# posgraph/coupe.optical_flow_based_deep_video_stabilization

Hardware: AMD Instinct MI355X
Metric: stabilised frame-pairs/sec @512x512 (higher is better)
Workload: dtype f32; 1 GPU; batch=8 512x512x27 frame stacks per GPU: FlowNetS-pyramid forward (5 flows) + flow resize/scale + tf_warp at 512x512; batch_per_gpu=8, height=512, width=512, cin=27, all_gather=False, vgg16_trunk=False, st_warp=none, plan_flags=0, plan_batch=0, full=False

## Files before the change

### coupe/optical_flow_based_deep_video_stabilization_amd/csrc/conv1_bf16x3.hip

```cpp
#include "rowwin_tile.h"

namespace vstab {

typedef unsigned u32x2 __attribute__((ext_vector_type(2)));
typedef unsigned u32x4 __attribute__((ext_vector_type(4)));
typedef __bf16 bf16x4 __attribute__((ext_vector_type(4)));
typedef __bf16 bf16x8 __attribute__((ext_vector_type(8)));

template <int NWIN4, int MB>
__global__ __launch_bounds__(256) void conv1_bf16x3_kernel(const RowWinParams p)
{
    extern __shared__ __attribute__((aligned(16))) char smem[];
    unsigned *planes = reinterpret_cast<unsigned *>(smem);

    const RowWinTile<MB> t = rowwin_tile<MB>(p);
    const int tid = t.tid, wm = t.wm, wn = t.wn, li = t.li, lh = t.lh;
    const int oy = t.row, pix_step = t.pix_step;

    f32x4 wv[NWIN4];
    auto load_window = [&](int ky) { rowwin_load_window(t, p, oy, ky, wv); };
    const int plane_w = p.WLEN >> 1;
    auto split_store = [&]() {
#pragma unroll
        for (int j = 0; j < NWIN4; ++j) {
            const int c4 = tid + 256 * j;
            if (4 * c4 < p.WLEN) {
                bf16x4 h, m, l;
#pragma unroll
                for (int e = 0; e < 4; ++e) {
                    const float x = wv[j][e];
                    h[e] = (__bf16)x;
                    const float r1 = x - (float)h[e];
                    m[e] = (__bf16)r1;
                    const float r2 = r1 - (float)m[e];
                    l[e] = (__bf16)r2;
                }
                *reinterpret_cast<u32x2 *>(planes + 2 * c4) = __builtin_bit_cast(u32x2, h);
                *reinterpret_cast<u32x2 *>(planes + plane_w + 2 * c4) = __builtin_bit_cast(u32x2, m);
                *reinterpret_cast<u32x2 *>(planes + 2 * plane_w + 2 * c4) = __builtin_bit_cast(u32x2, l);
            }
        }
    };

    const int KG = p.SEGP >> 4;
    const int NG = p.KH * KG;
    const unsigned *bbase = reinterpret_cast<const unsigned *>(p.wpk) + (wn * 32 + li) * 8 + lh * 4;
    auto load_b = [&](u32x4 (&b)[3], int G) {
        const unsigned *s = bbase + (long long)(G < NG ? G : NG - 1) * (3 * 512);
#pragma unroll
        for (int q = 0; q < 3; ++q) b[q] = *reinterpret_cast<const u32x4 *>(s + q * 512);
    };
    const int a_w0 = (pix_step * (wm * 32 * MB + li) + p.w_a + 8 * lh) >> 1;
    const int a_w1 = a_w0 + ((pix_step * 32) >> 1);
    auto load_a = [&](u32x4 (&a)[3 * MB], int g) {
#pragma unroll
        for (int mb = 0; mb < MB; ++mb)
#pragma unroll
            for (int q = 0; q < 3; ++q) {
                const unsigned *s = planes + q * plane_w + (mb ? a_w1 : a_w0) + 8 * g;
                u32x4 v;
                v.x = s[0]; v.y = s[1]; v.z = s[2]; v.w = s[3];
                a[mb * 3 + q] = v;
            }
    };

    f32x16 acc[MB];
#pragma unroll
    for (int a = 0; a < MB; ++a)
#pragma unroll
        for (int r = 0; r < 16; ++r) acc[a][r] = 0.f;

    auto mma = [&](const u32x4 (&a)[3 * MB], const u32x4 (&b)[3]) {
        constexpr int PA[6] = {2, 1, 0, 1, 0, 0}, PB[6] = {0, 1, 2, 0, 1, 0};
#pragma unroll
        for (int t = 0; t < 6; ++t)
#pragma unroll
            for (int mb = 0; mb < MB; ++mb)
                acc[mb] = __builtin_amdgcn_mfma_f32_32x32x16_bf16(__builtin_bit_cast(bf16x8, a[mb * 3 + PA[t]]),
                                                                  __builtin_bit_cast(bf16x8, b[PB[t]]), acc[mb], 0, 0, 0);
    };

    u32x4 a0[3 * MB], a1[3 * MB], b0[3], b1[3];
    load_window(0);
    load_b(b0, 0);
    split_store();
    __syncthreads();
    int G = 0;
    for (int ky = 0; ky < p.KH; ++ky) {
        const bool more = ky + 1 < p.KH;
        if (more) load_window(ky + 1);
        load_a(a0, 0);
        __builtin_amdgcn_sched_barrier(0);
        for (int g = 0; g < KG; g += 2, G += 2) {
            load_a(a1, g + 1);
            load_b(b1, G + 1);
            __builtin_amdgcn_sched_barrier(0);
            mma(a0, b0);
            __builtin_amdgcn_sched_barrier(0);
            if (g + 2 < KG) load_a(a0, g + 2);
            load_b(b0, G + 2);
            __builtin_amdgcn_sched_barrier(0);
            mma(a1, b1);
            __builtin_amdgcn_sched_barrier(0);
        }
        if (more) {
            __syncthreads();
            split_store();
            __syncthreads();
        }
    }

    rowwin_epilogue(t, p, acc, oy, reinterpret_cast<float *>(smem));
}

hipError_t conv1_bf16x3_set_attributes()
{
    return rowwin_set_lds_limits(conv1_bf16x3_kernel<7, 2>, 3 * 7 * 1024 * 2, conv1_bf16x3_kernel<4, 1>, 3 * 4 * 1024 * 2);
}

hipError_t launch_conv1_bf16x3(const RowWinParams &p, hipStream_t stream, hipEvent_t ev_start, hipEvent_t ev_stop)
{
    if (!conv1_bf16x3_geometry_ok(p)) return hipErrorInvalidValue;
    RowWinParams q = p;
    q.asm_loop = 0;
    q.stream_rows = 0;
    return rowwin_launch(q, conv1_bf16x3_kernel<7, 2>, conv1_bf16x3_kernel<4, 1>, (size_t)3 * p.WLEN * 2, stream, ev_start, ev_stop);
}

}
```

### coupe/optical_flow_based_deep_video_stabilization_amd/csrc/conv_desc.cpp

```cpp
#include <algorithm>
#include <cstring>

#include "conv_desc.h"

using namespace vstab;

namespace {
ConvParams desc_base(int B, int Hi, int Wi, int cs_in, const KLayout &L, int s_in, int s_out, int Ho, int Wo, int cout, int npad, int cs_out,
                     int c_off, int act, int nphase)
{
    ConvParams p;
    std::memset(&p, 0, sizeof p);
    p.B = B; p.Hi = Hi; p.Wi = Wi; p.Cs_in = cs_in;
    p.KH = L.KH; p.NSEG = L.NSEG; p.SEG = L.SEG; p.SEGP = L.SEGP; p.SEG_STRIDE = L.SEG_STRIDE;
    p.s_in = s_in; p.s_out = s_out; p.Ho = Ho; p.Wo = Wo; p.Cs_out = cs_out; p.c_off = c_off;
    p.N = cout; p.Npad = npad; p.act = act; p.nphase = nphase; p.ksplit = 1;
    p.in_bytes = (unsigned)std::min<long long>((long long)B * Hi * Wi * cs_in * 4, 0xFFFFFFFFLL);
    p.w_bytes = (unsigned)std::min<long long>((long long)L.ktiles() * npad * 128, 0xFFFFFFFFLL);
    return p;
}

void set_phase(ConvParams &p, int k, int Hg, int Wg, int off_y, int off_x, int o_y, int o_x)
{
    ConvPhase &ph = p.ph[k];
    ph.Hg = Hg; ph.Wg = Wg; ph.M = p.B * Hg * Wg;
    ph.off_y = off_y; ph.off_x = off_x; ph.o_y = o_y; ph.o_x = o_x;
    ph.w_off = (long long)k * ((long long)p.KH * p.NSEG * (p.SEGP / 32) * p.Npad * 32);
    p.Mmax = std::max(p.Mmax, ph.M);
}
}

ConvParams conv_desc_phase(int B, int Hi, int Wi, int cin, int cs_in, int kh, int kw, int s_in, const ConvGrid &g, int Ho, int Wo, int cout,
                           int npad, int cs_out, int c_off, int act)
{
    ConvParams p = desc_base(B, Hi, Wi, cs_in, conv_layout(kh, kw, cin, cs_in), s_in, g.s_out, Ho, Wo, cout, npad, cs_out, c_off, act, 1);
    set_phase(p, 0, g.Hg, g.Wg, g.off_y, g.off_x, g.o_y, g.o_x);
    return p;
}

ConvParams conv_desc_parity4(int B, int Hi, int Wi, int cin, int cs_in, int taps, const int off[2], int Ho, int Wo, int cout, int npad,
                             int cs_out, int c_off, int act)
{
    ConvParams p = desc_base(B, Hi, Wi, cs_in, conv_layout(taps, taps, cin, cs_in), 1, 2, Ho, Wo, cout, npad, cs_out, c_off, act, 4);
    for (int py = 0; py < 2; ++py)
        for (int px = 0; px < 2; ++px) set_phase(p, py * 2 + px, (Ho - py + 1) / 2, (Wo - px + 1) / 2, off[py], off[px], py, px);
    return p;
}

ConvParams conv_desc_planes(int B, int P, int pitch, int Wi, const int *Hg, const int *Wg, int cs_in, int cout)
{
    ConvParams p = desc_base(B, P * pitch, Wi, cs_in, klayout_run(1, 1, cs_in), 1, 1, P * pitch, Wi, cout, cout, cout, 0, 0, P);
    for (int q = 0; q < P; ++q) set_phase(p, q, Hg[q], Wg[q], q * pitch, 0, q * pitch, 0);
    return p;
}

ConvParams conv_desc_wino_gemm(int B, int H, int W, int cin, int cout)
{
    int Hg[16], Wg[16];
    for (int q = 0; q < 16; ++q) { Hg[q] = (H + 1) / 2; Wg[q] = (W + 1) / 2; }
    return conv_desc_planes(B, 16, Hg[0], Wg[0], Hg, Wg, cin, cout);
}

ConvParams conv_desc_wdec_gemm(int B, const WdecGeom &g, int cs_in, int cout)
{
    int Hg[9], Wg[9];
    for (int q = 0; q < 9; ++q) { Hg[q] = g.nty[q / 3]; Wg[q] = g.ntx[q % 3]; }
    return conv_desc_planes(B, 9, g.NTy, g.NTx, Hg, Wg, cs_in, 4 * cout);
}

RowWinDesc rowwin_desc(int B, int H, int W, int cin, int k, int stride, int pad, int Ho, int Wo, int cout, int npad, int cs_out, int c_off,
                       int act)
{
    RowWinDesc d;
    std::memset(&d, 0, sizeof d);
    RowWinParams &r = d.main;
    r.in_bytes = (unsigned)std::min<long long>((long long)B * H * W * cin * 4, 0xFFFFFFFFLL);
    r.B = B; r.Hi = H; r.Wi = W; r.Cs_in = cin; r.KH = k;
    r.SEGP = rowwin_segp(-pad, k, cin);
    r.s_in = stride; r.off_y = -pad;
    r.e_off = -pad * cin - rowwin_lead(-pad, cin);
    r.w_a = ((r.e_off % 4) + 4) % 4;
    r.Ho = Ho; r.Wo = Wo; r.Cs_out = cs_out; r.c_off = c_off; r.N = cout; r.Npad = npad; r.act = act;
    auto tile = [](RowWinParams &q, int MB) { q.MB = MB; q.WLEN = round_up(q.s_in * q.Cs_in * (64 * MB - 1) + q.w_a + q.SEGP, 4); };
    tile(r, rowwin_mb(B, Ho, Wo));
    d.ok = rowwin_geometry_ok(r);
    const int rem = Wo % 128;
    if (d.ok && r.MB == 2 && Wo > 128 && rem >= 1 && rem <= 64) {
        RowWinParams &t = d.tail;
        t = r;
        tile(t, 1);
        t.ox_base = (Wo / 128) * 128; t.ntile_x = 1;
        d.two = rowwin_geometry_ok(t);
        if (d.two) r.ntile_x = Wo / 128;
    }
    return d;
}
```

### coupe/optical_flow_based_deep_video_stabilization_amd/csrc/conv_desc.h

```cpp
#pragma once
#include "vstab_internal.h"

inline vstab::ConvTile default_tile(int cout)
{
    return cout >= 128 ? vstab::TILE_128x128 : (cout > 32 ? vstab::TILE_128x64 : vstab::TILE_128x32);
}
inline int tile_cols(vstab::ConvTile t)
{
    return (t == vstab::TILE_128x128 || t == vstab::TILE_64x128) ? 128 : ((t == vstab::TILE_128x64 || t == vstab::TILE_64x64) ? 64 : 32);
}
inline int padded_cols(int cout, vstab::ConvTile t) { return vstab::round_up(cout, tile_cols(t)); }
inline int padded_cols(int cout) { return padded_cols(cout, default_tile(cout)); }

inline vstab::KLayout conv_layout(int kh, int kw, int cin, int cs_in)
{
    return cs_in == cin ? vstab::klayout_run(kh, kw, cs_in) : vstab::klayout_tap(kh, kw, cin, cs_in);
}

struct ConvGrid { int Hg, Wg, off_y, off_x, s_out, o_y, o_x; };
vstab::ConvParams conv_desc_phase(int B, int Hi, int Wi, int cin, int cs_in, int kh, int kw, int s_in, const ConvGrid &g, int Ho, int Wo,
                                  int cout, int npad, int cs_out, int c_off, int act);
inline vstab::ConvParams conv_desc_plain(int B, int Hi, int Wi, int cin, int cs_in, int k, int stride, int pad, int Ho, int Wo, int cout,
                                         int npad, int cs_out, int c_off, int act)
{
    return conv_desc_phase(B, Hi, Wi, cin, cs_in, k, k, stride, ConvGrid{Ho, Wo, -pad, -pad, 1, 0, 0}, Ho, Wo, cout, npad, cs_out, c_off, act);
}

vstab::ConvParams conv_desc_parity4(int B, int Hi, int Wi, int cin, int cs_in, int taps, const int off[2], int Ho, int Wo, int cout, int npad,
                                    int cs_out, int c_off, int act);

vstab::ConvParams conv_desc_planes(int B, int P, int pitch, int Wi, const int *Hg, const int *Wg, int cs_in, int cout);
vstab::ConvParams conv_desc_wino_gemm(int B, int H, int W, int cin, int cout);
vstab::ConvParams conv_desc_wdec_gemm(int B, const vstab::WdecGeom &g, int cs_in, int cout);

struct RowWinDesc { vstab::RowWinParams main, tail; bool ok, two; };
RowWinDesc rowwin_desc(int B, int H, int W, int cin, int k, int stride, int pad, int Ho, int Wo, int cout, int npad, int cs_out, int c_off,
                       int act);
```

### coupe/optical_flow_based_deep_video_stabilization_amd/csrc/conv_rowwin.hip

```cpp
#include "rowwin_tile.h"

namespace vstab {

typedef float f32x2 __attribute__((ext_vector_type(2)));
typedef int i32x4 __attribute__((ext_vector_type(4)));
#include "conv_kloop_gfx950.inc"

template <int NWIN4, int MB>
__global__ __launch_bounds__(256) void conv_rowwin_kernel(const RowWinParams p)
{
    extern __shared__ __attribute__((aligned(16))) char smem[];
    float *win = reinterpret_cast<float *>(smem);

    const RowWinTile<MB> t = rowwin_tile<MB>(p);
    const int tid = t.tid, wm = t.wm, wn = t.wn, li = t.li, lh = t.lh;
    const int stream_r = (MB == 2 && p.asm_loop) ? p.stream_rows : 0;
    const int stream_s = 1;
    int oy = stream_r > 0 ? t.row * stream_r : t.row;
    const int ox0 = t.ox0, n = t.n, pix_step = t.pix_step, row_floats = t.row_floats;

    f32x4 wv[NWIN4];
    auto load_window = [&](int ky) { rowwin_load_window(t, p, oy, ky, wv); };
    constexpr int ASM_BUF = MB == 2 ? VSTAB_ROWWIN_BUF_BYTES : VSTAB_ROWWIN1_BUF_BYTES;
    const int wstride = p.asm_loop ? ASM_BUF / 4 : p.WLEN;
    auto store_window = [&](int buf) {
        float *d = win + buf * wstride;
#pragma unroll
        for (int j = 0; j < NWIN4; ++j) {
            const int c4 = tid + 256 * j;
            if (4 * c4 < p.WLEN) *reinterpret_cast<f32x4 *>(d + 4 * c4) = wv[j];
        }
    };

    const float *bbase = p.wpk + (long long)(wn * 32 + li) * 32 + lh * 4;
    const int ktile_stride = p.Npad * 32;
    f32x4 b0[4], b1[4];
    const int KT = p.KH * (p.SEGP >> 5);
    auto load_b = [&](f32x4 (&dst)[4], int kt) {
        const float *s = bbase + (long long)(kt < KT ? kt : KT - 1) * ktile_stride;
#pragma unroll
        for (int q = 0; q < 4; ++q) dst[q] = *reinterpret_cast<const f32x4 *>(s + q * 8);
    };

    f32x16 acc[MB];
#pragma unroll
    for (int a = 0; a < MB; ++a)
#pragma unroll
        for (int r = 0; r < 16; ++r) acc[a][r] = 0.f;

    const int kpr = p.SEGP >> 5;
    const int a_off0 = pix_step * (wm * 32 * MB + li) + p.w_a + 2 * lh;
    const int a_off1 = a_off0 + pix_step * 32;

    auto compute = [&](const float *w, int kc, const f32x4 (&b)[4]) {
        const float *wa0 = w + a_off0 + 32 * kc, *wa1 = w + a_off1 + 32 * kc;
#pragma unroll
        for (int r = 0; r < 8; ++r) {
            const f32x2 a0 = *reinterpret_cast<const f32x2 *>(wa0 + 4 * r);
            f32x2 a1 = a0;
            if (MB == 2) a1 = *reinterpret_cast<const f32x2 *>(wa1 + 4 * r);
#pragma unroll
            for (int j = 0; j < 2; ++j) {
                const int s = 2 * r + j;
                const float bv = b[s >> 2][s & 3];
                acc[0] = __builtin_amdgcn_mfma_f32_32x32x2f32(a0[j], bv, acc[0], 0, 0, 0);
                if (MB == 2) acc[MB - 1] = __builtin_amdgcn_mfma_f32_32x32x2f32(a1[j], bv, acc[MB - 1], 0, 0, 0);
            }
        }
    };

    load_window(0);
    store_window(0);
    if (p.asm_loop) {
        {
            __syncthreads();
            const unsigned lds0 = (unsigned)(size_t)(__attribute__((address_space(3))) void *)win;
            unsigned a0c = lds0 + (unsigned)a_off0 * 4u, a1c = lds0 + (unsigned)a_off1 * 4u;
            unsigned a0n = a0c + ASM_BUF, a1n = a1c + ASM_BUF;
            const unsigned vb = (unsigned)((wn * 32 + li) * 32 + lh * 4) * 4u;
            unsigned w[7];
#pragma unroll
            for (int j = 0; j < 7; ++j) w[j] = ROWWIN_OOB;
#pragma unroll
            for (int j = 0; j < NWIN4; ++j) {
                int g;
                if (rowwin_chunk(t, p, j, g)) w[j] = (unsigned)g * 4u;
            }
            const unsigned long long ain = (unsigned long long)(size_t)p.in, awt = (unsigned long long)(size_t)p.wpk;
            i32x4 din, dwt;
            din.x = __builtin_amdgcn_readfirstlane((int)(unsigned)ain);
            din.y = __builtin_amdgcn_readfirstlane((int)((unsigned)(ain >> 32) & 0xffffu));
            din.z = __builtin_amdgcn_readfirstlane((int)p.in_bytes);
            din.w = 0x00020000;
            dwt.x = __builtin_amdgcn_readfirstlane((int)(unsigned)awt);
            dwt.y = __builtin_amdgcn_readfirstlane((int)((unsigned)(awt >> 32) & 0xffffu));
            dwt.z = __builtin_amdgcn_readfirstlane(KT * ktile_stride * 4);
            dwt.w = 0x00020000;
            const int wave_u = __builtin_amdgcn_readfirstlane(tid) >> 6;
            const int m_cur = __builtin_amdgcn_readfirstlane((int)lds0 + wave_u * 1024);
            int m_n = m_cur + ASM_BUF;
            const int m_x = m_cur ^ m_n;
            int s_iy = oy * p.s_in + p.off_y + 1;
            int s_soff = ((n * p.Hi + s_iy) * p.Wi) * p.Cs_in * 4;
            int s_koff = 0, s_nrows = p.KH - 1;
            unsigned v_t0, v_t1;
            long long s_mask;
            if (MB == 2 && stream_r > 0) {
                const unsigned long long aout = (unsigned long long)(size_t)p.out;
                i32x4 dout;
                dout.x = __builtin_amdgcn_readfirstlane((int)(unsigned)aout);
                dout.y = __builtin_amdgcn_readfirstlane((int)((unsigned)(aout >> 32) & 0xffffu));
                dout.z = __builtin_amdgcn_readfirstlane((int)((unsigned)p.B * (unsigned)p.Ho * (unsigned)p.Wo * (unsigned)p.Cs_out * 4u));
                dout.w = 0x00020000;
                const unsigned vout = (unsigned)((wm * 64 + 4 * lh) * p.Cs_out + p.c_off + wn * 32 + li) * 4u;
                const float bias_l = p.bias[wn * 32 + li];
                const float slope = p.act == 1 ? 0.1f : (p.act == 0 ? 1.0f : 0.0f);
                int s_ntiles = stream_r, s_obase = (((n * p.Ho + oy) * p.Wo + ox0) * p.Cs_out) * 4, s_st;
                float o[32];
                asm volatile(VSTAB_ROWWIN_STREAM_ASM_KPR6
                             : [a0c] "+v"(a0c), [a1c] "+v"(a1c), [a0n] "+v"(a0n), [a1n] "+v"(a1n),
                               [mn] "+s"(m_n), [iy] "+s"(s_iy), [soff] "+s"(s_soff), [koff] "+s"(s_koff), [nrows] "+s"(s_nrows), [ntiles] "+s"(s_ntiles),
                               [obase] "+s"(s_obase), [st] "=&s"(s_st), [vt0] "=&v"(v_t0), [vt1] "=&v"(v_t1), [mask] "=&s"(s_mask),
                               [o0] "=&v"(o[0]), [o1] "=&v"(o[1]), [o2] "=&v"(o[2]), [o3] "=&v"(o[3]), [o4] "=&v"(o[4]), [o5] "=&v"(o[5]), [o6] "=&v"(o[6]),
                               [o7] "=&v"(o[7]), [o8] "=&v"(o[8]), [o9] "=&v"(o[9]), [o10] "=&v"(o[10]), [o11] "=&v"(o[11]), [o12] "=&v"(o[12]),
                               [o13] "=&v"(o[13]), [o14] "=&v"(o[14]), [o15] "=&v"(o[15]), [o16] "=&v"(o[16]), [o17] "=&v"(o[17]), [o18] "=&v"(o[18]),
                               [o19] "=&v"(o[19]), [o20] "=&v"(o[20]), [o21] "=&v"(o[21]), [o22] "=&v"(o[22]), [o23] "=&v"(o[23]), [o24] "=&v"(o[24]),
                               [o25] "=&v"(o[25]), [o26] "=&v"(o[26]), [o27] "=&v"(o[27]), [o28] "=&v"(o[28]), [o29] "=&v"(o[29]), [o30] "=&v"(o[30]),
                               [o31] "=&v"(o[31])
                             : [vb] "v"(vb), [w0] "v"(w[0]), [w1] "v"(w[1]), [w2] "v"(w[2]), [w3] "v"(w[3]), [w4] "v"(w[4]), [w5] "v"(w[5]), [w6] "v"(w[6]),
                               [din] "s"(din), [dwt] "s"(dwt), [mx] "s"(m_x), [hi] "s"(p.Hi), [rowbytes] "s"(row_floats * 4), [kstride] "s"(ktile_stride * 4),
                               [bias] "v"(bias_l), [slope] "s"(slope), [cs4] "s"(p.Cs_out * 4), [ostep] "s"(stream_s * p.Wo * p.Cs_out * 4), [vout] "v"(vout),
                               [dout] "s"(dout), [fwd] "s"(stream_s * p.s_in - p.KH)
                             : "memory", "scc", VSTAB_ROWWIN_STREAM_CLOBBERS);
#pragma unroll
                for (int r = 0; r < 16; ++r) { acc[0][r] = o[r]; acc[MB - 1][r] = o[16 + r]; }
                oy += (stream_r - 1) * stream_s;
            } else if constexpr (MB == 1) {
                asm volatile(VSTAB_ROWWIN1_ASM_KPR6
                             : [c0] "+a"(acc[0]), [a0c] "+v"(a0c), [a0n] "+v"(a0n),
                               [mn] "+s"(m_n), [iy] "+s"(s_iy), [soff] "+s"(s_soff), [koff] "+s"(s_koff), [nrows] "+s"(s_nrows),
                               [vt0] "=&v"(v_t0), [vt1] "=&v"(v_t1), [mask] "=&s"(s_mask)
                             : [vb] "v"(vb), [w0] "v"(w[0]), [w1] "v"(w[1]), [w2] "v"(w[2]), [w3] "v"(w[3]),
                               [din] "s"(din), [dwt] "s"(dwt), [mx] "s"(m_x), [hi] "s"(p.Hi), [rowbytes] "s"(row_floats * 4), [kstride] "s"(ktile_stride * 4)
                             : "memory", "scc", VSTAB_ROWWIN1_CLOBBERS);
                (void)a1c; (void)a1n;
            } else
            asm volatile(VSTAB_ROWWIN_ASM_KPR6
                         : [c0] "+a"(acc[0]), [c1] "+a"(acc[MB - 1]), [a0c] "+v"(a0c), [a1c] "+v"(a1c), [a0n] "+v"(a0n), [a1n] "+v"(a1n),
                           [mn] "+s"(m_n), [iy] "+s"(s_iy), [soff] "+s"(s_soff), [koff] "+s"(s_koff), [nrows] "+s"(s_nrows),
                           [vt0] "=&v"(v_t0), [vt1] "=&v"(v_t1), [mask] "=&s"(s_mask)
                         : [vb] "v"(vb), [w0] "v"(w[0]), [w1] "v"(w[1]), [w2] "v"(w[2]), [w3] "v"(w[3]), [w4] "v"(w[4]), [w5] "v"(w[5]), [w6] "v"(w[6]),
                           [din] "s"(din), [dwt] "s"(dwt), [mx] "s"(m_x), [hi] "s"(p.Hi), [rowbytes] "s"(row_floats * 4), [kstride] "s"(ktile_stride * 4)
                         : "memory", "scc", VSTAB_ROWWIN_CLOBBERS);
        }
    } else {
    load_b(b0, 0);
    __syncthreads();
    int buf = 0, kt = 0;
    for (int ky = 0; ky < p.KH; ++ky) {
        const bool more = ky + 1 < p.KH;
        if (more) load_window(ky + 1);
        __builtin_amdgcn_sched_barrier(0);
        const float *w = win + buf * p.WLEN;
        int kc = 0;
        for (; kc + 1 < kpr; kc += 2, kt += 2) {
            load_b(b1, kt + 1);
            __builtin_amdgcn_sched_barrier(0);
            compute(w, kc, b0);
            load_b(b0, kt + 2);
            __builtin_amdgcn_sched_barrier(0);
            compute(w, kc + 1, b1);
        }
        if (kc < kpr) {
            load_b(b1, kt + 1);
            __builtin_amdgcn_sched_barrier(0);
            compute(w, kc, b0);
#pragma unroll
            for (int q = 0; q < 4; ++q) b0[q] = b1[q];
            ++kt;
        }
        if (more) {
            store_window(buf ^ 1);
            __syncthreads();
            buf ^= 1;
        }
    }
    }

    rowwin_epilogue(t, p, acc, oy, win);
}

hipError_t rowwin_set_attributes()
{
    return rowwin_set_lds_limits(conv_rowwin_kernel<7, 2>, 2 * 7 * 1024 * 4, conv_rowwin_kernel<4, 1>, 2 * 4 * 1024 * 4);
}

hipError_t launch_conv_rowwin(const RowWinParams &p, hipStream_t stream, hipEvent_t ev_start, hipEvent_t ev_stop)
{
    const int ntx = rowwin_xtiles(p);
    if (!rowwin_geometry_ok(p) || ntx < 0) return hipErrorInvalidValue;
    RowWinParams q = p;
    q.asm_loop = ((p.SEGP >> 5) == 6 && p.KH >= 1 && 4 * p.WLEN <= (p.MB == 2 ? VSTAB_ROWWIN_BUF_BYTES : VSTAB_ROWWIN1_BUF_BYTES)) ? 1 : 0;
#ifdef VSTAB_NO_ASM_KLOOP
    q.asm_loop = 0;
#endif
    q.stream_rows = 0;
    if (q.asm_loop && p.MB == 2 && p.KH == 7 && p.N == 64 && p.act >= 0 && p.act <= 2 && p.ox_base + ntx * 128 <= p.Wo &&
        (unsigned long long)p.B * p.Ho * p.Wo * p.Cs_out * 4ull < 0x80000000ull) {
        const double F = 0.08;
        const long long cols = (long long)ntx * p.B;
        double best = (double)((cols * p.Ho + 511) / 512) * (1.0 + F);
        for (int R = 2; R <= 32 && R <= p.Ho; ++R) {
            if (p.Ho % R) continue;
            const long long wgs = cols * (p.Ho / R);
            const double c = wgs <= 256 ? 0.53 * R + F : (double)((wgs + 511) / 512) * (R + F);
            if (c < best * 0.995) { best = c; q.stream_rows = R; }
        }
    }
#ifdef VSTAB_NO_ROWWIN_STREAM
    q.stream_rows = 0;
#endif
    const size_t lds2 = q.asm_loop ? (size_t)2 * (p.MB == 2 ? VSTAB_ROWWIN_BUF_BYTES : VSTAB_ROWWIN1_BUF_BYTES) : (size_t)2 * p.WLEN * 4;
    return rowwin_launch(q, conv_rowwin_kernel<7, 2>, conv_rowwin_kernel<4, 1>, lds2, stream, ev_start, ev_stop);
}

}
```

### coupe/optical_flow_based_deep_video_stabilization_amd/csrc/flownet_forward.cpp

```cpp
#include <cmath>
#include <cstdlib>
#include <memory>

#include "flownet_plan.h"

using namespace vstab;

static const char *UP_NAME[4] = {"upsample6_5", "upsample5_4", "upsample4_3", "upsample3_2"};

extern "C" int vstab_load_weights(vstab_ctx *ctx, const vstab_tensor *t, int count)
{
    if (!ctx) return fail(nullptr, VSTAB_E_STATE, "vstab_load_weights: ctx is NULL");
    if (!t || count <= 0) return fail(ctx, VSTAB_E_WEIGHTS, "vstab_load_weights: no tensors");
    const vstab_tensor *w1 = find(t, count, "1/W_conv2d");
    if (!w1 || w1->ndim != 4) return fail(ctx, VSTAB_E_WEIGHTS, "missing variable 1/W_conv2d");
    const int cin = w1->shape[2];
    if (cin < 1 || cin > 4096) return fail(ctx, VSTAB_E_WEIGHTS, "1/W_conv2d: bad Cin %d", cin);

    std::vector<float> host;
    auto reserve = [&](size_t n) { size_t o = (host.size() + 63) / 64 * 64; host.resize(o + n, 0.f); return o; };
    std::vector<double> scale;
    auto need = [&](const std::string &name, std::initializer_list<int> s) -> const vstab_tensor * {
        const vstab_tensor *x = find(t, count, name);
        return shape_is(x, s) ? x : nullptr;
    };
#define NEED(var, name, ...)                                                                   \
    const vstab_tensor *var = need(name, {__VA_ARGS__});                                        \
    if (!var) return fail(ctx, VSTAB_E_WEIGHTS, "missing or mis-shaped variable %s", std::string(name).c_str());

    for (int i = 0; i < 10; ++i) {
        const Layer &e = NET[i];
        const int ci = i == 0 ? cin : e.cin;
        const int cs_in = i == 0 ? cin : in_buf(e).cs;
        const std::string n = e.name + 4;
        NEED(W, n + "/W_conv2d", e.k, e.k, ci, e.cout)
        NEED(b, n + "/b_conv2d", e.cout)
        NEED(beta, n + "/beta", e.cout)
        NEED(mean, n + "/moving_mean", e.cout)
        NEED(var, n + "/moving_variance", e.cout)
        const int npad = padded_cols(e.cout);
        const KLayout L = conv_layout(e.k, e.k, ci, cs_in);
        scale.assign(npad, 1.0);
        ctx->enc_b[i] = reserve(npad);
        fold_bn(b->data, beta->data, mean->data, var->data, e.cout, npad, scale.data(), host.data() + ctx->enc_b[i]);
        ctx->enc_w[i] = reserve((size_t)L.ktiles() * npad * 32);
        pack_conv(W->data, scale.data(), e.k, e.k, ci, cs_in, e.cout, npad, L, host.data() + ctx->enc_w[i]);
        if (e.k == 3 && e.s == 1 && (ci & 31) == 0 && (e.cout & 127) == 0) {
            ctx->wino_w[i] = reserve((size_t)16 * (ci / 32) * e.cout * 32);
            pack_winograd(W->data, scale.data(), ci, e.cout, e.cout, host.data() + ctx->wino_w[i]);
        }
        if (i == 0) {
            const int lead = rowwin_lead(-e.p, cin), segp = rowwin_segp(-e.p, e.k, cin);
            ctx->enc0_rw = reserve((size_t)e.k * (segp / 32) * npad * 32);
            pack_conv_rowwin(W->data, scale.data(), e.k, e.k, cin, e.cout, npad, lead, segp, host.data() + ctx->enc0_rw);
            ctx->enc0_b3 = 0;
            if (npad == 64) {
                ctx->enc0_b3 = reserve((size_t)e.k * (segp / 16) * 3 * 64 * 16 / 2);
                pack_conv1_bf16x3(W->data, scale.data(), e.k, e.k, cin, e.cout, lead, segp, reinterpret_cast<uint16_t *>(host.data() + ctx->enc0_b3));
            }
        }
    }
    for (int l = 0; l < 4; ++l) {
        const Layer &d = dec_layer(l);
        const std::string n = d.name;
        const int co = d.cout, ci = d.cin, cs = in_buf(d).cs;
        NEED(W, n + "/W_deconv2d", 4, 4, co, ci)
        NEED(b, n + "/b_deconv2d", co)
        NEED(beta, n + "_bn/beta", co)
        NEED(mean, n + "_bn/moving_mean", co)
        NEED(var, n + "_bn/moving_variance", co)
        const int npad = padded_cols(co);
        scale.assign(npad, 1.0);
        ctx->dec_b[l] = reserve(npad);
        fold_bn(b->data, beta->data, mean->data, var->data, co, npad, scale.data(), host.data() + ctx->dec_b[l]);
        ctx->dec_w[l] = reserve(4 * (size_t)klayout_deconv(cs).ktiles() * npad * 32);
        pack_deconv(W->data, scale.data(), ci, cs, co, npad, host.data() + ctx->dec_w[l]);
        ctx->wdec_w[l] = 0;
        if (l <= 2) {
            ctx->wdec_w[l] = reserve(9 * (size_t)klayout_run(1, 1, cs).ktiles() * 4 * co * 32);
            pack_wdec(W->data, scale.data(), ci, cs, co, host.data() + ctx->wdec_w[l]);
        }

        const std::string u = UP_NAME[l];
        NEED(uw, u + "/W_deconv2d", 4, 4, 2, 2)
        NEED(ub, u + "/b_deconv2d", 2)
        std::memcpy(ctx->up[l].w, uw->data, sizeof(float) * 64);
        ctx->up[l].b[0] = ub->data[0]; ctx->up[l].b[1] = ub->data[1];
    }
    for (int l = 0; l < 4; ++l) {
        const Layer &h = head_layer(l);
        const std::string n = h.name;
        NEED(W, n + "/W_conv2d", 3, 3, h.cin, 2)
        NEED(b, n + "/b_conv2d", 2)
        ctx->pred_w[l] = reserve((size_t)klayout_run(1, 1, in_buf(h).cs).ktiles() * 32 * 32);
        pack_predict2_table(W->data, h.cin, in_buf(h).cs, 32, host.data() + ctx->pred_w[l]);
        ctx->pred_b[l] = reserve(4);
        host[ctx->pred_b[l]] = b->data[0]; host[ctx->pred_b[l] + 1] = b->data[1];
    }
    {
        NEED(W, "predict2/W_conv2d", 3, 3, NET[14].cin, 2)
        NEED(b, "predict2/b_conv2d", 2)
        ctx->tab_b = reserve(32);
        ctx->tab_wp = reserve((size_t)200 * 32);
        pack_predict2_panel(W->data, NET[14].cin, 200, host.data() + ctx->tab_wp);
        ctx->zero_b = reserve(2048);
        ctx->pred2_b = reserve(4);
        host[ctx->pred2_b] = b->data[0]; host[ctx->pred2_b + 1] = b->data[1];
    }
#undef NEED

    HIP_TRY(ctx, hipSetDevice(ctx->device));
    if (ctx->dev_weights) { (void)hipFree(ctx->dev_weights); ctx->dev_weights = nullptr; }
    ctx->loaded = false;
    hipError_t e = hipMalloc(reinterpret_cast<void **>(&ctx->dev_weights), host.size() * sizeof(float));
    if (e != hipSuccess) return fail(ctx, VSTAB_E_NOMEM, "hipMalloc(%zu bytes of packed weights): %s", host.size() * 4, hipGetErrorString(e));
    HIP_TRY(ctx, hipMemcpy(ctx->dev_weights, host.data(), host.size() * sizeof(float), hipMemcpyHostToDevice));
    ctx->dev_weight_floats = host.size();
    ctx->cin = cin;
    ctx->loaded = true;
    return VSTAB_OK;
}

struct FusedTail { const float *frame; float *outflow; float *warped; int oh, ow; bool fused; const uint8_t *frame8; uint8_t *out8; };
static int forward_chunk(vstab_ctx *ctx, const float *feats, int B, int H, int W, int Cin, float *pf6, float *pf5,
                         float *pf4, float *pf3, float *pf2, void *workspace, size_t workspace_bytes, void *stream_, FusedTail *tail);
static const char *conv_kernel_name(ConvTile t, bool vec4);
static const char *dual_kernel_name(ConvTile t);
static int forward_impl(vstab_ctx *ctx, const float *feats, int B, int H, int W, int Cin, float *pf6, float *pf5, float *pf4, float *pf3,
                        float *pf2, void *workspace, size_t workspace_bytes, void *stream_, FusedTail *tail);

extern "C" int vstab_flownets_forward(vstab_ctx *ctx, const float *feats, int B, int H, int W, int Cin, float *pf6,
                                      float *pf5, float *pf4, float *pf3, float *pf2, void *workspace,
                                      size_t workspace_bytes, void *stream_)
{
    return forward_impl(ctx, feats, B, H, W, Cin, pf6, pf5, pf4, pf3, pf2, workspace, workspace_bytes, stream_, nullptr);
}

static int forward_impl(vstab_ctx *ctx, const float *feats, int B, int H, int W, int Cin, float *pf6, float *pf5, float *pf4, float *pf3,
                        float *pf2, void *workspace, size_t workspace_bytes, void *stream_, FusedTail *tail)
{
    if (!ctx) return fail(nullptr, VSTAB_E_STATE, "forward: ctx is NULL");
    if (!ctx->loaded) return fail(ctx, VSTAB_E_STATE, "forward: vstab_load_weights has not been called");
    if (Cin != ctx->cin) return fail(ctx, VSTAB_E_SHAPE, "forward: feats has %d channels, weights expect %d", Cin, ctx->cin);
    if (!feats || !pf6 || !pf5 || !pf4 || !pf3 || !pf2 || !workspace) return fail(ctx, VSTAB_E_STATE, "forward: NULL buffer");
    int eh[10], ew[10];
    if (B < 1 || !level_sizes(H, W, eh, ew)) return fail(ctx, VSTAB_E_SHAPE, "forward: unsupported problem %dx%dx%dx%d", B, H, W, Cin);
    const PlanPin pin = pin_of(ctx);
    if (pin.batch > 0 && B > pin.batch) return fail(ctx, VSTAB_E_SHAPE, "forward: batch %d exceeds the pinned plan batch %d (vstab_set_plan_batch)", B, pin.batch);
    const int chunk = chunk_size(pin, B, H, W, Cin);
    if (chunk < 1) return fail(ctx, VSTAB_E_SHAPE, "forward: one %dx%dx%d sample exceeds the 2 GiB tensor limit", H, W, Cin);
    bool all_fused = tail != nullptr && (chunk >= B || ((size_t)tail->oh * tail->ow * 4) % 16 == 0);
    for (int b0 = 0; b0 < B; b0 += chunk) {
        const int bc = std::min(chunk, B - b0);
        FusedTail t{};
        if (tail && all_fused) {
            const size_t px = (size_t)b0 * tail->oh * tail->ow;
            t = FusedTail{tail->frame ? tail->frame + px * 3 : nullptr, tail->outflow ? tail->outflow + px * 2 : nullptr,
                          tail->warped ? tail->warped + px * 3 : nullptr, tail->oh, tail->ow, false,
                          tail->frame8 ? tail->frame8 + px * 3 : nullptr, tail->out8 ? tail->out8 + px * 3 : nullptr};
        }
        const int rc = forward_chunk(ctx, feats + (size_t)b0 * H * W * Cin, bc, H, W, Cin,
                                     pf6 + (size_t)b0 * eh[9] * ew[9] * 2, pf5 + (size_t)b0 * eh[7] * ew[7] * 2,
                                     pf4 + (size_t)b0 * eh[5] * ew[5] * 2, pf3 + (size_t)b0 * eh[3] * ew[3] * 2,
                                     pf2 + (size_t)b0 * (H - 2) * (W - 2) * 2, workspace, workspace_bytes, stream_, (tail && all_fused) ? &t : nullptr);
        if (rc != VSTAB_OK) return rc;
        if (tail && all_fused && !t.fused) {
            if (b0 != 0) return fail(ctx, VSTAB_E_ALIGN, "stabilise: chunk %d of the batch misses the fused tail's alignment", b0 / chunk);
            all_fused = false;
        }
    }
    if (tail) tail->fused = all_fused;
    return VSTAB_OK;
}

static int conv1_rowwin(vstab_ctx *ctx, bool bf16x3, const float *feats, int B, int H, int W, int Cin, int Ho, int Wo, int N, int Npad,
                        float *out, int cs_out, int c_off, unsigned *tickets, hipStream_t stream, hipEvent_t ev_a, hipEvent_t ev_b,
                        const char **kname, bool *launched)
{
    const Layer &e = NET[0];
    const float *dw = ctx->dev_weights;
    *launched = false;
    RowWinDesc d = rowwin_desc(B, H, W, Cin, e.k, e.s, e.p, Ho, Wo, N, Npad, cs_out, c_off, 1);
    if (!d.ok || ((uintptr_t)feats & 15) != 0) return VSTAB_OK;
    const bool b3 = bf16x3 && ctx->enc0_b3 != 0 && conv1_bf16x3_geometry_ok(d.main);
    RowWinParams &r = d.main, &t = d.tail;
    r.in = t.in = feats; r.out = t.out = out; r.bias = t.bias = dw + ctx->enc_b[0];
    r.wpk = t.wpk = dw + (b3 ? ctx->enc0_b3 : ctx->enc0_rw);
    auto launch1 = [&](const RowWinParams &q, hipEvent_t a, hipEvent_t b) {
        return b3 ? launch_conv1_bf16x3(q, stream, a, b) : launch_conv_rowwin(q, stream, a, b);
    };
    if (tickets) { r.clear_words = tickets; r.clear_n = SKINNY_MAX_TILES; }
    *launched = true;
    if (d.two) {
        HIP_TRY(ctx, launch1(r, ev_a, nullptr));
        HIP_TRY(ctx, launch1(t, nullptr, ev_b));
        *kname = b3 ? "conv1_bf16x3_kernel<7, 2> + <4, 1> tail" : "conv_rowwin_kernel<7, 2> + <4, 1> tail";
        return VSTAB_OK;
    }
    HIP_TRY(ctx, launch1(r, ev_a, ev_b));
    if (b3) *kname = r.MB == 2 ? "conv1_bf16x3_kernel<7, 2>" : "conv1_bf16x3_kernel<4, 1>";
    else *kname = r.MB == 2 ? "conv_rowwin_kernel<7, 2>" : "conv_rowwin_kernel<4, 1>";
    return VSTAB_OK;
}

extern "C" int vstab_conv1_forward(vstab_ctx *ctx, const float *feats, int B, int H, int W, int Cin, float *out, int cs_out, int c_off,
                                   void *stream_)
{
    if (!ctx) return fail(nullptr, VSTAB_E_STATE, "conv1_forward: ctx is NULL");
    if (!ctx->loaded) return fail(ctx, VSTAB_E_STATE, "conv1_forward: vstab_load_weights has not been called");
    if (Cin != ctx->cin) return fail(ctx, VSTAB_E_SHAPE, "conv1_forward: feats has %d channels, weights expect %d", Cin, ctx->cin);
    if (!feats || !out) return fail(ctx, VSTAB_E_STATE, "conv1_forward: NULL buffer");
    const PlanPin pin = pin_of(ctx);
    std::unique_ptr<Plan> pl(new (std::nothrow) Plan);
    if (!pl) return fail(ctx, VSTAB_E_NOMEM, "conv1_forward: out of host memory");
    if (B < 1 || !make_plan(B, H, W, Cin, *pl, &pin)) return fail(ctx, VSTAB_E_SHAPE, "conv1_forward: unsupported problem %dx%dx%dx%d", B, H, W, Cin);
    const ConvParams &p = pl->cp[0];
    if (c_off < 0 || cs_out < c_off + p.N || (long long)B * p.Ho * p.Wo * cs_out * 4 >= 0x80000000LL)
        return fail(ctx, VSTAB_E_SHAPE, "conv1_forward: output slice %d + %d of %d channels", c_off, p.N, cs_out);
    if (((uintptr_t)feats & 15) || ((uintptr_t)out & 3)) return fail(ctx, VSTAB_E_ALIGN, "conv1_forward: feats must be 16-byte aligned");
    const char *kname = nullptr;
    bool launched = false;
    const int rc = conv1_rowwin(ctx, pl->conv1_bf16x3, feats, B, H, W, Cin, p.Ho, p.Wo, p.N, p.Npad, out, cs_out, c_off, nullptr,
                                (hipStream_t)stream_, nullptr, nullptr, &kname, &launched);
    if (rc != VSTAB_OK) return rc;
    if (!launched) return fail(ctx, VSTAB_E_SHAPE, "conv1_forward: the row-window kernels do not take this geometry");
    return VSTAB_OK;
}

static int forward_chunk(vstab_ctx *ctx, const float *feats, int B, int H, int W, int Cin, float *pf6, float *pf5,
                         float *pf4, float *pf3, float *pf2, void *workspace, size_t workspace_bytes, void *stream_, FusedTail *tail)
{
    Plan pl;
    const PlanPin pin = pin_of(ctx);
    if (!make_plan(B, H, W, Cin, pl, &pin)) return fail(ctx, VSTAB_E_SHAPE, "forward: unsupported problem %dx%dx%dx%d", B, H, W, Cin);
    if (workspace_bytes < pl.total) return fail(ctx, VSTAB_E_NOMEM, "forward: workspace %zu < %zu bytes", workspace_bytes, pl.total);
    if (((uintptr_t)workspace & 255) != 0) return fail(ctx, VSTAB_E_ALIGN, "forward: workspace must be 256-byte aligned");
    if (((uintptr_t)feats & 15) || ((uintptr_t)pf6 & 7) || ((uintptr_t)pf5 & 7) || ((uintptr_t)pf4 & 7) ||
        ((uintptr_t)pf3 & 7) || ((uintptr_t)pf2 & 7))
        return fail(ctx, VSTAB_E_ALIGN, "forward: feats must be 16-byte and flows 8-byte aligned");
    hipStream_t stream = (hipStream_t)stream_;
    char *ws = (char *)workspace;
    auto buf = [&](int b) { return (float *)(ws + pl.off[b]); };
    const float *dw = ctx->dev_weights;
    unsigned *tickets = reinterpret_cast<unsigned *>(buf(B_TICKETS));
    bool any_tickets = false;
    for (int i = 0; i < 14; ++i) any_tickets = any_tickets || (pl.skinny[i] && pl.cp[i].ksplit > 1);
    bool tickets_cleared = !any_tickets;

    hipEvent_t *ev = nullptr;
    if (ctx->prof) {
        const size_t need = (size_t)(ctx->prof_forwards + 1) * 30;
        while (ctx->prof_ev.size() < need) {
            hipEvent_t e;
            HIP_TRY(ctx, hipEventCreate(&e));
            ctx->prof_ev.push_back(e);
        }
        ev = ctx->prof_ev.data() + (size_t)ctx->prof_forwards * 30;
        for (int i = 0; i < 15; ++i) {
            const ConvParams &p = pl.cp[i];
            double mac = 0;
            if (i < 10 && pl.wino[i]) mac = 16.0 * pl.wcp[i].Mmax * NET[i].cin * p.N;
            else if (i < 10) mac = (double)p.ph[0].M * NET[i].k * NET[i].k * (i == 0 ? Cin : NET[i].cin) * p.N;
            else if (i < 14 && pl.wdec[i - 10]) {
                for (int k = 0; k < 9; ++k) mac += (double)pl.wdcp[i - 10].ph[k].M * NET[i].cin * 4.0 * p.N;
            }
            else if (i < 14) mac = (double)B * p.Ho * p.Wo * 4.0 * NET[i].cin * p.N;
            else mac = (double)p.ph[0].M * 194.0 * 18.0;
            ctx->prof_flops[i] += 2.0 * mac;
            double dmac = mac;
            if (i < 10 && pl.wino[i]) dmac = (double)p.ph[0].M * 9.0 * NET[i].cin * p.N;
            if (i >= 10 && i < 14 && pl.wdec[i - 10]) dmac = (double)B * p.Ho * p.Wo * 4.0 * NET[i].cin * p.N;
            ctx->prof_flops_direct[i] += 2.0 * dmac;
        }
    }
#define PROF_NAME(slot, name) do { if (ev) ctx->prof_kernel[slot] = (name); } while (0)
#define EV_A(slot) (ev ? ev[2 * (slot)] : nullptr)
#define EV_B(slot) (ev ? ev[2 * (slot) + 1] : nullptr)

    static const char *const HEAD_RANGE[4] = {"predict_flow6+upsample6_5", "predict_flow5+upsample5_4", "predict_flow4+upsample4_3", "predict_flow3+upsample3_2"};
    TraceRange whole_range("flownetS_pyramid");
    for (int i = 0; i < 10; ++i) {
        const Layer &e = NET[i];
        TraceRange layer_range(e.name);
        ConvParams p = pl.cp[i];
        if (i == 0) {
            const char *kname = nullptr;
            bool launched = false;
            const int rc = conv1_rowwin(ctx, pl.conv1_bf16x3, feats, B, H, W, Cin, p.Ho, p.Wo, p.N, p.Npad, buf(B_CONV1), p.Cs_out, 0,
                                        tickets_cleared ? nullptr : tickets, stream, EV_A(0), EV_B(0), &kname, &launched);
            if (rc != VSTAB_OK) return rc;
            if (launched) { tickets_cleared = true; PROF_NAME(0, kname); continue; }
        }
        if (!tickets_cleared) { HIP_TRY(ctx, hipMemsetAsync(tickets, 0, pl.bytes[B_TICKETS], stream)); tickets_cleared = true; }
        if (pl.wino[i]) {
            ConvParams q = pl.wcp[i];
            const int cin_i = e.cin;
            HIP_TRY(ctx, launch_wino_input(buf(e.in), B, pl.eh[i], pl.ew[i], in_buf(e).cs, 0, cin_i, buf(B_WINO_V), stream));
            q.in = buf(B_WINO_V); q.out = buf(B_WINO_M);
            q.wpk = dw + ctx->wino_w[i]; q.bias = dw + ctx->zero_b; q.partial = buf(B_PARTIAL);
            const int T_i = ((pl.eh[i] + 1) / 2) * ((pl.ew[i] + 1) / 2);
            const int P_i = wino_gemm_stream_positions(B, T_i, cin_i, e.cout);
            if (P_i > 0) {
                HIP_TRY(ctx, launch_wino_gemm_stream(q.in, q.wpk, q.out, B, T_i, cin_i, e.cout, P_i, stream, EV_A(i), EV_B(i)));
                PROF_NAME(i, "wino_gemm_stream_kernel");
            } else {
                HIP_TRY(ctx, launch_conv(q, pl.wtile[i], true, stream, EV_A(i), EV_B(i)));
                PROF_NAME(i, conv_kernel_name(pl.wtile[i], true));
            }
            HIP_TRY(ctx, launch_wino_output(buf(B_WINO_M), B, pl.eh[i], pl.ew[i], e.cout, dw + ctx->enc_b[i], 1, buf(e.out),
                                            out_buf(e).cs, 0, stream));
            continue;
        }
        p.in = e.in < 0 ? feats : buf(e.in);
        p.out = buf(e.out);
        p.wpk = dw + ctx->enc_w[i];
        p.bias = dw + ctx->enc_b[i];
        p.partial = buf(B_PARTIAL);
        if (pl.skinny[i]) {
            HIP_TRY(ctx, launch_conv_skinny(p, tickets, stream, EV_A(i), EV_B(i)));
            PROF_NAME(i, "conv_skinny_kernel<1, 4>");
            continue;
        }
        HIP_TRY(ctx, launch_conv(p, pl.tile[i], pl.vec4[i], stream, EV_A(i), EV_B(i)));
        PROF_NAME(i, conv_kernel_name(pl.tile[i], pl.vec4[i]));
    }
    float *pfs[5] = {pf6, pf5, pf4, pf3, pf2};
    for (int l = 0; l < 4; ++l) {
        const float *prev = l == 0 ? nullptr : pfs[l - 1];
        const Layer &d = dec_layer(l);
        const int ph_ = l == 0 ? 0 : pl.eh[LVL_ENC[l - 1]], pw_ = l == 0 ? 0 : pl.ew[LVL_ENC[l - 1]];
        const int oh = pl.eh[LVL_ENC[l + 1]], ow = pl.ew[LVL_ENC[l + 1]];
        ConvParams pd = pl.cp[10 + l], pt = pl.cp[15 + l];
        pd.in = buf(d.in); pd.out = buf(d.out);
        pd.wpk = dw + ctx->dec_w[l]; pd.bias = dw + ctx->dec_b[l]; pd.partial = buf(B_PARTIAL);
        const size_t dec_slab = pd.ksplit > 1 ? (size_t)pd.nphase * pd.ksplit * pd.Mmax * pd.Npad : 0;
        pt.in = buf(head_layer(l).in); pt.out = buf(head_layer(l).out);
        pt.wpk = dw + ctx->pred_w[l]; pt.bias = dw + ctx->tab_b; pt.partial = buf(B_PARTIAL) + dec_slab;
        const float *tsrc = pt.ksplit > 1 ? pt.partial : pt.out;
        const bool fuse = !(pin.flags & VSTAB_PLAN_NO_DUAL) && !pl.skinny[10 + l];
        auto head = [&](const float *taps, const ConvParams *combine, const WdecOutArgs *wdec) {
            return launch_predict_up(taps, pt.ksplit, (long long)pt.Mmax * pt.Npad, B, pt.Hi, pt.Wi, dw + ctx->pred_b[l], prev, ph_, pw_, pfs[l],
                                     ctx->up[l], buf(d.out), oh, ow, out_buf(d).cs, out_buf(d).c - 2, stream, combine, wdec);
        };
        auto dual = [&](const ConvParams &a, ConvTile ta) -> int {
            const hipError_t e = launch_conv_dual(a, ta, pt, pl.tile[15 + l], stream, EV_A(10 + l), EV_B(10 + l));
            if (e == hipErrorNotSupported) {
                HIP_TRY(ctx, launch_conv(pt, pl.tile[15 + l], true, stream, nullptr, nullptr, false));
                HIP_TRY(ctx, launch_conv(a, ta, true, stream, EV_A(10 + l), EV_B(10 + l), false));
                PROF_NAME(10 + l, conv_kernel_name(ta, true));
            } else {
                HIP_TRY(ctx, e);
                PROF_NAME(10 + l, dual_kernel_name(ta));
            }
            return VSTAB_OK;
        };
        if (fuse && pl.wdec[l]) {
            const WdecGeom &g = pl.wdg[l];
            {
                TraceRange r2(d.name);
                HIP_TRY(ctx, launch_wdec_input(pd.in, B, pd.Hi, pd.Wi, pd.Cs_in, buf(B_WINO_V), g, stream));
                ConvParams q = pl.wdcp[l];
                q.in = buf(B_WINO_V); q.out = buf(B_WINO_M); q.wpk = dw + ctx->wdec_w[l]; q.bias = dw + ctx->zero_b; q.partial = buf(B_PARTIAL);
                pt.partial = buf(B_PARTIAL);
                if (const int rc = dual(q, pl.wdtile[l])) return rc;
            }
            TraceRange r3(HEAD_RANGE[l]);
            const WdecOutArgs wo{buf(B_WINO_M), pd.N / 4, dw + ctx->dec_b[l], 1, buf(d.out), pd.Ho, pd.Wo, pd.Cs_out, pd.c_off, g};
            HIP_TRY(ctx, head(pt.ksplit > 1 ? pt.partial : pt.out, nullptr, &wo));
            continue;
        }
        if (fuse) {
            {
                TraceRange r2(d.name);
                if (const int rc = dual(pd, pl.tile[10 + l])) return rc;
            }
            TraceRange r3(HEAD_RANGE[l]);
            HIP_TRY(ctx, head(tsrc, &pd, nullptr));
            continue;
        }
        {
            TraceRange head_range(HEAD_RANGE[l]);
            HIP_TRY(ctx, launch_conv(pt, pl.tile[15 + l], true, stream, nullptr, nullptr, false));
            HIP_TRY(ctx, head(tsrc, nullptr, nullptr));
        }
        TraceRange layer_range(d.name);
        if (pl.skinny[10 + l]) {
            HIP_TRY(ctx, launch_conv_skinny(pd, tickets, stream, EV_A(10 + l), EV_B(10 + l)));
            PROF_NAME(10 + l, "conv_skinny_kernel<1, 4>");
        } else {
            HIP_TRY(ctx, launch_conv(pd, pl.tile[10 + l], true, stream, EV_A(10 + l), EV_B(10 + l)));
            PROF_NAME(10 + l, conv_kernel_name(pl.tile[10 + l], true));
        }
    }
    {
        TraceRange layer_range("predict_flow2");
        ConvParams p = pl.cp[14];
        p.in = buf(B_CONCAT2); p.out = buf(B_T);
        const long long M2 = (long long)B * pl.eh[1] * pl.ew[1];
        if (!tap_panel_applicable(M2, p.Cs_in, p.in, p.out)) return fail(ctx, VSTAB_E_SHAPE, "predict_flow2 tap table: unsupported geometry");
        HIP_TRY(ctx, launch_tap_panel(p.in, M2, dw + ctx->tab_wp, p.out, stream, EV_A(14), EV_B(14)));
        PROF_NAME(14, "tap_panel_kernel");
        hipError_t te = hipErrorNotSupported;
        if (tail && !(pin.flags & VSTAB_PLAN_NO_TAIL)) {
            TraceRange tail_range("predict_flow2 gather+flow_glue+tf_warp");
            if (tail->frame8)
                te = launch_pf2_glue_warp_u8(buf(B_T), B, pl.eh[1], pl.ew[1], dw + ctx->pred2_b, pf3, pl.eh[3], pl.ew[3], pf2, H, W, tail->frame8,
                                             tail->outflow, tail->out8, tail->oh, tail->ow, stream);
            else
                te = launch_pf2_glue_warp(buf(B_T), B, pl.eh[1], pl.ew[1], dw + ctx->pred2_b, pf3, pl.eh[3], pl.ew[3], pf2, H, W, tail->frame,
                                          tail->outflow, tail->warped, tail->oh, tail->ow, stream);
            if (te != hipSuccess && te != hipErrorNotSupported) HIP_TRY(ctx, te);
            tail->fused = te == hipSuccess;
        }
        if (te != hipSuccess) HIP_TRY(ctx, launch_pf2(buf(B_T), B, pl.eh[1], pl.ew[1], dw + ctx->pred2_b, pf3, pl.eh[3], pl.ew[3], pf2, H, W, stream));
    }
#undef EV_A
#undef EV_B
#undef PROF_NAME
    if (ev) ctx->prof_forwards++;
    return VSTAB_OK;
}

static const char *conv_kernel_name(ConvTile t, bool vec4)
{
    const bool dma = conv_uses_lds_dma(t, vec4);
#define VSTAB_KN(shape) (vec4 ? (dma ? "conv_mfma_kernel<" shape ", true, true>" : "conv_mfma_kernel<" shape ", true, false>") \
                              : (dma ? "conv_mfma_kernel<" shape ", false, true>" : "conv_mfma_kernel<" shape ", false, false>"))
    switch (t) {
    case TILE_128x128: return VSTAB_KN("128, 128, 2, 2");
    case TILE_128x64: return VSTAB_KN("128, 64, 2, 2");
    case TILE_64x128: return VSTAB_KN("64, 128, 1, 4");
    case TILE_64x64: return VSTAB_KN("64, 64, 2, 2");
    case TILE_256x32: return VSTAB_KN("256, 32, 4, 1");
    default: return VSTAB_KN("128, 32, 4, 1");
    }
#undef VSTAB_KN
}

static const char *dual_kernel_name(ConvTile t)
{
    const bool dma = conv_uses_lds_dma(t, true);
#define VSTAB_DN(shape) (dma ? "conv_dual_kernel: conv_mfma_kernel<" shape ", true, true> + <128, 32> tap table" \
                             : "conv_dual_kernel: conv_mfma_kernel<" shape ", true, false> + <128, 32> tap table")
    switch (t) {
    case TILE_128x128: return VSTAB_DN("128, 128, 2, 2");
    case TILE_128x64: return VSTAB_DN("128, 64, 2, 2");
    case TILE_64x128: return VSTAB_DN("64, 128, 1, 4");
    case TILE_64x64: return VSTAB_DN("64, 64, 2, 2");
    case TILE_256x32: return VSTAB_DN("256, 32, 4, 1");
    default: return VSTAB_DN("128, 32, 4, 1");
    }
#undef VSTAB_DN
}

extern "C" int vstab_profile_kernel_name(vstab_ctx *ctx, int slot, char *buf, int cap)
{
    if (!ctx || !buf || cap < 1 || slot < 0 || slot > 14) return fail(ctx, VSTAB_E_STATE, "profile_kernel_name: bad argument");
    std::snprintf(buf, (size_t)cap, "%s", ctx->prof_kernel[slot] ? ctx->prof_kernel[slot] : "");
    return VSTAB_OK;
}

extern "C" int vstab_profile_enable(vstab_ctx *ctx, int enable)
{
    if (!ctx) return fail(nullptr, VSTAB_E_STATE, "profile_enable: ctx is NULL");
    ctx->prof = enable != 0;
    return VSTAB_OK;
}

extern "C" int vstab_profile_reset(vstab_ctx *ctx)
{
    if (!ctx) return fail(nullptr, VSTAB_E_STATE, "profile_reset: ctx is NULL");
    ctx->prof_forwards = 0;
    for (double &f : ctx->prof_flops) f = 0;
    for (double &f : ctx->prof_flops_direct) f = 0;
    return VSTAB_OK;
}

extern "C" int vstab_profile_read(vstab_ctx *ctx, double *ms_sum15, double *flops15, int *n_forwards)
{
    if (!ctx || !ms_sum15 || !flops15 || !n_forwards) return fail(ctx, VSTAB_E_STATE, "profile_read: NULL argument");
    for (int i = 0; i < 15; ++i) { ms_sum15[i] = 0; flops15[i] = ctx->prof_flops[i]; }
    for (int f = 0; f < ctx->prof_forwards; ++f)
        for (int i = 0; i < 15; ++i) {
            float ms = 0.f;
            HIP_TRY(ctx, hipEventElapsedTime(&ms, ctx->prof_ev[(size_t)f * 30 + 2 * i], ctx->prof_ev[(size_t)f * 30 + 2 * i + 1]));
            ms_sum15[i] += ms;
        }
    *n_forwards = ctx->prof_forwards;
    return VSTAB_OK;
}

extern "C" int vstab_profile_read_direct(vstab_ctx *ctx, double *flops15)
{
    if (!ctx || !flops15) return fail(ctx, VSTAB_E_STATE, "profile_read_direct: NULL argument");
    for (int i = 0; i < 15; ++i) flops15[i] = ctx->prof_flops_direct[i];
    return VSTAB_OK;
}

extern "C" int vstab_stabilise_originalsize(vstab_ctx *ctx, const float *feats, int B, int H, int W, int Cin, const float *frame, int oh,
                                            int ow, float *pf6, float *pf5, float *pf4, float *pf3, float *pf2, float *outflow,
                                            float *warped, void *workspace, size_t workspace_bytes, void *stream)
{
    if (!frame || !warped) return fail(ctx, VSTAB_E_STATE, "stabilise_originalsize: NULL buffer");
    if (oh < 1 || ow < 1) return fail(ctx, VSTAB_E_SHAPE, "stabilise_originalsize: bad output size");
    FusedTail tail{frame, outflow, warped, oh, ow, false, nullptr, nullptr};
    const bool try_fused = (((uintptr_t)frame | (uintptr_t)warped | (uintptr_t)outflow) & 15) == 0;
    const int rc = forward_impl(ctx, feats, B, H, W, Cin, pf6, pf5, pf4, pf3, pf2, workspace, workspace_bytes, stream, try_fused ? &tail : nullptr);
    if (rc != VSTAB_OK) return rc;
    if (tail.fused) return VSTAB_OK;
    const int rc2 = vstab_flow_glue_warp(pf2, B, H - 2, W - 2, frame, outflow, warped, oh, ow, 3, H, W, stream);
    if (rc2 != VSTAB_OK) adopt_last_error(ctx);
    return rc2;
}

extern "C" int vstab_clip_step(vstab_ctx *ctx, const uint8_t *const *slots8, const uint8_t *frame, int n, int net_h, int net_w, int oh, int ow,
                               float *feats, float *pf6, float *pf5, float *pf4, float *pf3, float *pf2, float *outflow, uint8_t *out,
                               uint8_t *ring_slot, void *workspace, size_t workspace_bytes, void *stream)
{
    if (!ctx) return fail(nullptr, VSTAB_E_STATE, "clip_step: ctx is NULL");
    if (!slots8 || !frame || !feats || !out || !ring_slot) return fail(ctx, VSTAB_E_STATE, "clip_step: NULL buffer");
    if (n < 1 || net_h < 3 || net_w < 4 || oh < 1 || ow < 1) return fail(ctx, VSTAB_E_SHAPE, "clip_step: bad shape");
    {
        const size_t fb = (size_t)n * oh * ow * 3, sb = (size_t)n * net_h * net_w * 3;
        auto overlap = [](const void *a, size_t na, const void *b, size_t nb) {
            const uintptr_t x = (uintptr_t)a, y = (uintptr_t)b;
            return x < y + nb && y < x + na;
        };
        if (overlap(out, fb, frame, fb) || overlap(ring_slot, sb, frame, fb) || overlap(ring_slot, sb, out, fb))
            return fail(ctx, VSTAB_E_STATE, "clip_step: out / ring_slot / frame must not overlap");
    }
    int rc = vstab_assemble_input_resized(slots8, frame, n, net_h, net_w, oh, ow, feats, stream);
    FusedTail tail{nullptr, outflow, nullptr, oh, ow, false, frame, out};
    const bool try_fused = (((uintptr_t)outflow & 7) | ((uintptr_t)out & 3)) == 0 && (long long)n * oh * ow < (1ll << 31) / 3;
    if (rc == VSTAB_OK) rc = forward_impl(ctx, feats, n, net_h, net_w, 27, pf6, pf5, pf4, pf3, pf2, workspace, workspace_bytes, stream, try_fused ? &tail : nullptr);
    else adopt_last_error(ctx);
    if (rc != VSTAB_OK) return rc;
    if (!tail.fused) rc = vstab_flow_glue_warp_u8(pf2, n, net_h - 2, net_w - 2, frame, outflow, out, oh, ow, net_h, net_w, stream);
    if (rc == VSTAB_OK) rc = vstab_resize_u8(out, n, oh, ow, ring_slot, net_h, net_w, stream);
    if (rc != VSTAB_OK) adopt_last_error(ctx);
    return rc;
}
```

### coupe/optical_flow_based_deep_video_stabilization_amd/csrc/flownet_plan.cpp

```cpp
#include <cmath>
#include <cstdlib>
#include <memory>
#include <new>

#include "flownet_plan.h"

using namespace vstab;

bool level_sizes(int H, int W, int *eh, int *ew)
{
    int h = H, w = W;
    for (int i = 0; i < 10; ++i) {
        h = (h + 2 * NET[i].p - NET[i].k) / NET[i].s + 1;
        w = (w + 2 * NET[i].p - NET[i].k) / NET[i].s + 1;
        if (h < 1 || w < 1) return false;
        eh[i] = h; ew[i] = w;
    }
    for (int l = 0; l < 4; ++l)
        if ((eh[LVL_ENC[l + 1]] + 1) / 2 != eh[LVL_ENC[l]] || (ew[LVL_ENC[l + 1]] + 1) / 2 != ew[LVL_ENC[l]]) return false;
    return H >= 3 && W >= 3;
}

static double split_cost_us(long long tiles, int KT, int ks, double slab_bytes, int BN, int BM, int *ks_eff_out)
{
    const double TAU2 = 4.2 * (BN >= 128 ? 1.0 : (BN == 64 ? 0.58 : 0.36)) * (BM == 64 ? 0.55 : 1.0);
    const double TAU1 = 0.525 * TAU2, T0 = 5.0;
    const double BW = slab_bytes * ((KT + ((KT + ks - 1) / ks) - 1) / ((KT + ks - 1) / ks)) > 16e6 ? 5.0e6 : 1.2e7;
    const int kts = (KT + ks - 1) / ks, ks_eff = (KT + kts - 1) / kts;
    const long long blocks = tiles * ks_eff, full = blocks / 512, rem = blocks % 512;
    double t = (double)full * (kts * TAU2 + T0);
    if (rem > 256) t += kts * TAU2 + T0;
    else if (rem > 0) t += kts * TAU1 + T0;
    if (ks_eff > 1) t += 6.0 + (2.0 * ks_eff + 1.0) * slab_bytes / BW;
    *ks_eff_out = ks_eff;
    return t;
}

static double best_split(const ConvParams &p, int BN, int BM, int *ks_out)
{
    const int KT = p.KH * p.NSEG * (p.SEGP / 32);
    const long long tiles = (long long)((p.Mmax + BM - 1) / BM) * (p.Npad / BN) * p.nphase;
    int best = 1, dummy;
    double best_t = split_cost_us(tiles, KT, 1, 0.0, BN, BM, &dummy);
    *ks_out = 1;
    if ((p.N & 3) != 0 || tiles >= 2048) return best_t;
    const double slab = (double)p.Mmax * p.nphase * p.Npad * 4.0;
    const int cap = std::min(64, std::max(1, KT / 3));
    for (int ks = 2; ks <= cap; ++ks) {
        int eff;
        const double t = split_cost_us(tiles, KT, ks, slab, BN, BM, &eff);
        if (eff != ks || slab * ks > 768e6) continue;
        if (t < best_t * 0.995) { best_t = t; best = ks; }
    }
    *ks_out = best;
    return best_t;
}

void choose_split(ConvParams &p, int BN, int BM)
{
    int ks;
    best_split(p, BN, BM, &ks);
    p.ksplit = ks;
}

ConvTile choose_tile_split(ConvParams &p, ConvTile tile, bool vec4)
{
    const int BN = tile == TILE_128x128 ? 128 : (tile == TILE_128x64 ? 64 : 32);
    int ks128;
    const double t128 = best_split(p, BN, 128, &ks128);
    p.ksplit = ks128;
    if (tile != TILE_128x128 || !vec4 || !conv_uses_lds_dma(tile, vec4)) return tile;
    int ks64;
    const double t64 = best_split(p, 128, 64, &ks64);
    if (t64 < 0.95 * t128) { p.ksplit = ks64; return TILE_64x128; }
    return tile;
}

bool choose_skinny(ConvParams &p, bool vec4, unsigned flags)
{
    if (flags & VSTAB_PLAN_NO_SKINNY) return false;
    if (!conv_skinny_applicable(p, vec4)) return false;
    p.ksplit = conv_skinny_split(p);
    return true;
}

bool wino_applies(int B, int H, int W, int cin, int cout)
{
#ifdef VSTAB_HARNESS
    static const bool wino_on = getenv("VSTAB_NO_WINOGRAD") == nullptr;
    if (!wino_on) return false;
#endif
    if ((cin & 31) || (cout & 127)) return false;
    const long long TH = (H + 1) / 2, TW = (W + 1) / 2;
    if ((long long)B * 16 * TH * TW * std::max(cin, cout) * 4 >= 0x80000000LL) return false;
#ifndef VSTAB_WINO_MIN_FLOPS
#define VSTAB_WINO_MIN_FLOPS 1.5e9
#endif
    return 32.0 * B * TH * TW * cin * cout >= VSTAB_WINO_MIN_FLOPS;
}

bool wdec_applies(int l, int B, const WdecGeom &g, int Hi, int Wi, int Ho, int Wo, int cs_in, int cout, double t_direct_us, int ks_direct, bool force,
                  ConvTile *tile_out)
{
    *tile_out = TILE_128x128;
#ifdef VSTAB_HARNESS
    static const bool wdec_on = getenv("VSTAB_NO_WDEC") == nullptr;
    if (!wdec_on) return false;
#endif
    if (l < 0 || l > 2 || (cs_in & 3) || ((4 * cout) & 127) || 4 * cout > 2048) return false;
    if ((long long)B * 9 * g.NTy * g.NTx * std::max(cs_in, 4 * cout) * 4 >= 0x80000000LL) return false;
    const int KT = round_up(cs_in, 32) / 32;
    double best = 1e30;
    for (int BM : {128, 64}) {
        long long tiles = 0;
        for (int i = 0; i < 3; ++i)
            for (int j = 0; j < 3; ++j) tiles += ((long long)B * g.nty[i] * g.ntx[j] + BM - 1) / BM;
        int eff;
        const double t = split_cost_us(tiles * (4 * cout / 128), KT, 1, 0.0, 128, BM, &eff);
        if (t < best) { best = t; *tile_out = BM == 128 ? TILE_128x128 : TILE_64x128; }
    }
    if (force) return true;
    const double plane = (double)B * g.NTy * g.NTx;
    const double bytes = 4.0 * ((double)B * Hi * Wi * cs_in + 9.0 * plane * cs_in + 9.0 * plane * 4.0 * cout + (double)B * Ho * Wo * cout);
#ifndef VSTAB_WDEC_MARGIN
#define VSTAB_WDEC_MARGIN 0.92
#endif
    if (ks_direct > 1) return false;
    return best + bytes / 4.5e6 + 3.0 < VSTAB_WDEC_MARGIN * t_direct_us;
}

bool fill_plain_conv(ConvParams &p, ConvTile &tile, bool &vec4, int B, int Hi, int Wi, int cin, int cs_in, int k, int stride,
                     int pad, int cout, int cs_out, int c_off, int act)
{
    const int Ho = (Hi + 2 * pad - k) / stride + 1, Wo = (Wi + 2 * pad - k) / stride + 1;
    if (Ho < 1 || Wo < 1 || cs_in < cin) return false;
    tile = default_tile(cout);
    p = conv_desc_plain(B, Hi, Wi, cin, cs_in, k, stride, pad, Ho, Wo, cout, padded_cols(cout), cs_out, c_off, act);
    vec4 = (cs_in % 4 == 0) && (p.SEG % 4 == 0);
    if (!vec4 && tile != TILE_128x64) return false;
    if ((long long)B * Hi * Wi * cs_in * 4 >= 0x80000000LL || (long long)B * Ho * Wo * cs_out * 4 >= 0x80000000LL) return false;
    tile = choose_tile_split(p, tile, vec4);
    return true;
}

static int max_chunk(int B, int H, int W, int Cin);

bool make_plan(int B, int H, int W, int Cin, Plan &pl, const PlanPin *pin)
{
    if (B < 1 || Cin < 1 || Cin > 4096) return false;
    pl.B = B; pl.H = H; pl.W = W; pl.Cin = Cin;
    if (!level_sizes(H, W, pl.eh, pl.ew)) return false;
    const unsigned flags = pin ? pin->flags : 0u;
    std::unique_ptr<Plan> ref;
    if (pin && pin->batch > 0) {
        if (B > pin->batch) return false;
        const int cmax = max_chunk(pin->batch, H, W, Cin);
        if (cmax < 1) return false;
        const int nch = (pin->batch + cmax - 1) / cmax, rb = (pin->batch + nch - 1) / nch;
        if (B > rb) return false;
        if (B != rb) {
            ref.reset(new (std::nothrow) Plan);
            PlanPin unpinned; unpinned.flags = flags;
            if (!ref || !make_plan(rb, H, W, Cin, *ref, &unpinned)) return false;
        }
    }
    const long long lim = (1LL << 29) - 1;
    if ((long long)B * H * W * Cin > lim) return false;

    for (int b = 0; b < N_BUF; ++b) {
        const long long n = (long long)B * pl.buf_h(b) * pl.buf_w(b) * BUFS[b].cs;
        if (n > lim) return false;
        pl.bytes[b] = (size_t)n * 4;
    }
    pl.bytes[B_TICKETS] = SKINNY_MAX_TILES * sizeof(unsigned);

    size_t partial_floats = 0;
    for (int i = 0; i < 10; ++i) {
        const Layer &e = NET[i];
        ConvParams &p = pl.cp[i];
        const int cin = i == 0 ? Cin : e.cin, cs_in = i == 0 ? Cin : in_buf(e).cs;
        p = conv_desc_plain(B, i == 0 ? H : pl.eh[i - 1], i == 0 ? W : pl.ew[i - 1], cin, cs_in, e.k, e.s, e.p, pl.eh[i], pl.ew[i], e.cout,
                            padded_cols(e.cout), out_buf(e).cs, e.c_off, 1);
        pl.tile[i] = default_tile(e.cout);
        pl.vec4[i] = (p.Cs_in % 4 == 0) && (p.SEG % 4 == 0);
        if (ref) { pl.tile[i] = ref->tile[i]; pl.skinny[i] = ref->skinny[i]; p.ksplit = ref->cp[i].ksplit; }
        else {
            pl.tile[i] = choose_tile_split(p, pl.tile[i], pl.vec4[i]);
            pl.skinny[i] = i > 0 && choose_skinny(p, pl.vec4[i], flags);
            if (pl.skinny[i]) pl.tile[i] = TILE_SKINNY;
        }
        if (p.ksplit > 1) partial_floats = std::max(partial_floats, (size_t)p.ksplit * p.Mmax * p.Npad);
    }
    pl.conv1_bf16x3 = ref ? ref->conv1_bf16x3
                          : (!(flags & VSTAB_PLAN_CONV1_FP32) && NET[0].cout == 64 && rowwin_segp(-NET[0].p, NET[0].k, Cin) <= 192);
    size_t wino_v = 0, wino_m = 0;
    for (int i = 0; i < 10; ++i) {
        pl.wino[i] = false;
        const Layer &e = NET[i];
        if (e.k != 3 || e.s != 1 || e.p != 1 || pl.skinny[i]) continue;
        if (ref ? !ref->wino[i] : (in_buf(e).cs != e.cin || !wino_applies(B, pl.eh[i], pl.ew[i], e.cin, e.cout))) continue;
        const int TH = (pl.eh[i] + 1) / 2, TW = (pl.ew[i] + 1) / 2;
        pl.wcp[i] = conv_desc_wino_gemm(B, pl.eh[i], pl.ew[i], e.cin, e.cout);
        {
            const long long t128 = 16LL * ((pl.wcp[i].Mmax + 127) / 128) * (e.cout / 128);
            pl.wtile[i] = t128 >= 1024 ? TILE_128x128 : TILE_128x64;
        }
        wino_v = std::max(wino_v, (size_t)B * 16 * TH * TW * e.cin);
        wino_m = std::max(wino_m, (size_t)B * 16 * TH * TW * e.cout);
        pl.wino[i] = true;
    }
    for (int l = 0; l < 4; ++l) {
        const Layer &d = dec_layer(l);
        ConvParams &p = pl.cp[10 + l];
        const int off[2] = {-1, 0};
        p = conv_desc_parity4(B, pl.buf_h(d.in), pl.buf_w(d.in), in_buf(d).cs, in_buf(d).cs, 2, off, pl.buf_h(d.out), pl.buf_w(d.out), d.cout,
                              padded_cols(d.cout), out_buf(d).cs, d.c_off, 1);
        pl.tile[10 + l] = default_tile(d.cout);
        pl.vec4[10 + l] = true;
        if (ref) { pl.tile[10 + l] = ref->tile[10 + l]; pl.skinny[10 + l] = ref->skinny[10 + l]; p.ksplit = ref->cp[10 + l].ksplit; }
        else {
            pl.tile[10 + l] = choose_tile_split(p, pl.tile[10 + l], true);
            pl.skinny[10 + l] = (flags & VSTAB_PLAN_NO_DUAL) ? choose_skinny(p, true, flags) : false;
            if (pl.skinny[10 + l]) pl.tile[10 + l] = TILE_SKINNY;
        }
        if (p.ksplit > 1) partial_floats = std::max(partial_floats, (size_t)p.nphase * p.ksplit * p.Mmax * p.Npad);
        pl.wdec[l] = false;
        pl.wdg[l] = wdec_geom(p.Hi, p.Wi, p.Ho, p.Wo);
        if (!(flags & (VSTAB_PLAN_NO_DUAL | VSTAB_PLAN_NO_WDEC)) && !pl.skinny[10 + l]) {
            const ConvTile dt = pl.tile[10 + l];
            int ks_d;
            ConvParams pd1 = p;
            const double t_direct = best_split(pd1, dt == TILE_128x64 ? 64 : 128, dt == TILE_64x128 ? 64 : 128, &ks_d);
            ConvTile wt;
            const bool on = wdec_applies(l, B, pl.wdg[l], p.Hi, p.Wi, p.Ho, p.Wo, p.Cs_in, p.N, t_direct, p.ksplit, (flags & VSTAB_PLAN_FORCE_WDEC) != 0, &wt);
            if (ref ? ref->wdec[l] : on) {
                const WdecGeom &g = pl.wdg[l];
                pl.wdcp[l] = conv_desc_wdec_gemm(B, g, p.Cs_in, p.N);
                pl.wdtile[l] = wt;
                wino_v = std::max(wino_v, (size_t)B * 9 * g.NTy * g.NTx * p.Cs_in);
                wino_m = std::max(wino_m, (size_t)B * 9 * g.NTy * g.NTx * 4 * p.N);
                pl.wdec[l] = true;
            }
        }
    }
    pl.bytes[B_WINO_V] = wino_v * 4;
    pl.bytes[B_WINO_M] = wino_m * 4;
    for (int i = 14; i < N_LAYER; ++i) {
        const Layer &t = NET[i];
        ConvParams &p = pl.cp[i];
        const int h = pl.buf_h(t.in), w = pl.buf_w(t.in), cs = in_buf(t).cs;
        p = conv_desc_plain(B, h, w, cs, cs, 1, 1, 0, h, w, 32, 32, out_buf(t).cs, 0, 0);
        pl.tile[i] = TILE_128x32; pl.vec4[i] = true; pl.skinny[i] = false;
        if (i == 14) continue;
        if (ref) p.ksplit = ref->cp[i].ksplit;
        else choose_split(p, 32);
        const ConvParams &d = pl.cp[i - 5];
        const size_t dec_slab = d.ksplit > 1 ? (size_t)d.nphase * d.ksplit * d.Mmax * d.Npad : 0;
        if (p.ksplit > 1) partial_floats = std::max(partial_floats, dec_slab + (size_t)p.ksplit * p.Mmax * p.Npad);
    }
    pl.bytes[B_PARTIAL] = partial_floats * 4;
    size_t off = 0;
    for (int b = 0; b < N_BUF; ++b) {
        pl.off[b] = off;
        off += (pl.bytes[b] + 255) / 256 * 256;
    }
    pl.total = off;
    return true;
}

static int max_chunk(int B, int H, int W, int Cin)
{
    Plan pl;
    return largest_fitting(B, [&](int b) { return make_plan(b, H, W, Cin, pl); });
}

int chunk_size(const PlanPin &pin, int B, int H, int W, int Cin)
{
    const int ref = pin.batch > 0 ? pin.batch : B;
    const int cmax = ref >= 1 ? max_chunk(ref, H, W, Cin) : 0;
    if (cmax < 1) return 0;
    const int nch = (ref + cmax - 1) / cmax;
    return std::min(B, (ref + nch - 1) / nch);
}

extern "C" int vstab_level_sizes(int H, int W, int32_t *hw20)
{
    int eh[10], ew[10];
    if (!hw20 || !level_sizes(H, W, eh, ew)) return fail(nullptr, VSTAB_E_SHAPE, "unsupported input size %dx%d", H, W);
    for (int i = 0; i < 10; ++i) { hw20[2 * i] = eh[i]; hw20[2 * i + 1] = ew[i]; }
    return VSTAB_OK;
}

extern "C" size_t vstab_workspace_bytes(int B, int H, int W, int Cin)
{
    Plan pl;
    const int chunk = B >= 1 ? max_chunk(B, H, W, Cin) : 0;
    if (chunk < 1 || !make_plan(chunk, H, W, Cin, pl)) { fail(nullptr, VSTAB_E_SHAPE, "unsupported problem %dx%dx%dx%d", B, H, W, Cin); return 0; }
    return pl.total;
}

extern "C" int vstab_set_plan_batch(vstab_ctx *ctx, int batch)
{
    if (!ctx) return fail(nullptr, VSTAB_E_STATE, "set_plan_batch: ctx is NULL");
    if (batch < 0) return fail(ctx, VSTAB_E_SHAPE, "set_plan_batch: batch must be >= 0 (0 = plan for the batch of each call)");
    ctx->plan_batch = batch;
    return VSTAB_OK;
}

extern "C" int vstab_set_plan_flags(vstab_ctx *ctx, unsigned flags)
{
    if (!ctx) return fail(nullptr, VSTAB_E_STATE, "set_plan_flags: ctx is NULL");
    if (flags & ~(unsigned)(VSTAB_PLAN_NO_SKINNY | VSTAB_PLAN_NO_DUAL | VSTAB_PLAN_NO_TAIL | VSTAB_PLAN_NO_WDEC | VSTAB_PLAN_FORCE_WDEC | VSTAB_PLAN_CONV1_FP32)) return fail(ctx, VSTAB_E_SHAPE, "set_plan_flags: unknown flag bits 0x%x", flags);
    ctx->plan_flags = flags;
    return VSTAB_OK;
}

extern "C" size_t vstab_workspace_bytes_ctx(const vstab_ctx *ctx, int B, int H, int W, int Cin)
{
    Plan pl;
    const PlanPin pin = pin_of(ctx);
    if (pin.batch > 0 && B > pin.batch) { fail(nullptr, VSTAB_E_SHAPE, "batch %d exceeds the pinned plan batch %d", B, pin.batch); return 0; }
    const int chunk = B >= 1 ? chunk_size(pin, B, H, W, Cin) : 0;
    if (chunk < 1 || !make_plan(chunk, H, W, Cin, pl, &pin)) { fail(nullptr, VSTAB_E_SHAPE, "unsupported problem %dx%dx%dx%d", B, H, W, Cin); return 0; }
    return pl.total;
}

static int workspace_layout_of(const PlanPin *pin, int chunk, int H, int W, int Cin, vstab_ws_entry *entries, int max_entries)
{
    Plan pl;
    if (!entries || chunk < 1 || !make_plan(chunk, H, W, Cin, pl, pin))
        return fail(nullptr, VSTAB_E_SHAPE, "unsupported problem %dx%dx%dx%d", chunk, H, W, Cin);
    int n = 0;
    for (int b = 0; b < N_BUF && n < max_entries; ++b) {
        vstab_ws_entry &e = entries[n++];
        std::memset(&e, 0, sizeof e);
        std::snprintf(e.name, sizeof e.name, "%s", BUFS[b].name);
        e.offset_bytes = (int64_t)pl.off[b];
        e.n = chunk; e.h = pl.buf_h(b); e.w = pl.buf_w(b); e.c = BUFS[b].c; e.c_stride = BUFS[b].cs;
        if (BUFS[b].level < 0) { e.n = 1; e.h = 1; e.w = (int32_t)std::min<size_t>(pl.bytes[b] / 4, 0x7fffffff); e.c = 1; e.c_stride = 1; }
    }
    return n;
}

extern "C" int vstab_workspace_layout(int B, int H, int W, int Cin, vstab_ws_entry *entries, int max_entries)
{
    return workspace_layout_of(nullptr, B >= 1 ? max_chunk(B, H, W, Cin) : 0, H, W, Cin, entries, max_entries);
}

extern "C" int vstab_workspace_layout_ctx(const vstab_ctx *ctx, int B, int H, int W, int Cin, vstab_ws_entry *entries, int max_entries)
{
    const PlanPin pin = pin_of(ctx);
    if (pin.batch > 0 && B > pin.batch) return fail(nullptr, VSTAB_E_SHAPE, "batch %d exceeds the pinned plan batch %d", B, pin.batch);
    return workspace_layout_of(&pin, B >= 1 ? chunk_size(pin, B, H, W, Cin) : 0, H, W, Cin, entries, max_entries);
}

static int put_desc(const ConvParams &p, int tile, int vec4, const Layer &L, bool alt_form, int32_t *out)
{
    const int v[26] = {p.B, p.Hi, p.Wi, p.Cs_in, p.KH, p.NSEG, p.SEG, p.SEGP, p.SEG_STRIDE, p.s_in, p.s_out, p.Ho, p.Wo,
                       p.Cs_out, p.c_off, p.N, p.Npad, p.act, p.nphase, p.ksplit, p.Mmax, tile, vec4, L.in, L.out, alt_form ? 1 : 0};
    for (int i = 0; i < 26; ++i) out[i] = v[i];
    for (int k = 0; k < p.nphase; ++k) {
        const ConvPhase &ph = p.ph[k];
        const int q[7] = {ph.Hg, ph.Wg, ph.M, ph.off_y, ph.off_x, ph.o_y, ph.o_x};
        for (int i = 0; i < 7; ++i) out[26 + 7 * k + i] = q[i];
    }
    return 26 + 7 * p.nphase;
}

extern "C" int vstab_host_layer_plan(int B, int H, int W, int Cin, int layer, int32_t *out, int cap)
{
    return vstab_host_layer_plan_pinned(0, 0u, B, H, W, Cin, layer, out, cap);
}

extern "C" int vstab_host_layer_plan_pinned(int plan_batch, unsigned flags, int B, int H, int W, int Cin, int layer, int32_t *out, int cap)
{
    Plan pl;
    PlanPin pin; pin.batch = plan_batch; pin.flags = flags;
    if (!out || layer < 0 || layer > 18 || plan_batch < 0 || !make_plan(B, H, W, Cin, pl, &pin))
        return fail(nullptr, VSTAB_E_SHAPE, "layer_plan: bad arguments");
    const ConvParams &p = pl.cp[layer];
    const int need = 26 + 7 * p.nphase;
    if (cap < need) return fail(nullptr, VSTAB_E_NOMEM, "layer_plan: need %d ints", need);
    return put_desc(p, (int)pl.tile[layer], (int)pl.vec4[layer], NET[layer],
                    (layer < 10 && pl.wino[layer]) || (layer >= 10 && layer < 14 && pl.wdec[layer - 10]), out);
}

extern "C" int vstab_host_wdec_plan(int B, int H, int W, int Cin, int l, int32_t *out, int cap)
{
    Plan pl;
    if (!out || l < 0 || l > 3 || !make_plan(B, H, W, Cin, pl)) return fail(nullptr, VSTAB_E_SHAPE, "wdec_plan: bad arguments");
    const ConvParams &d = pl.cp[10 + l];
    const WdecGeom g = wdec_geom(d.Hi, d.Wi, d.Ho, d.Wo);
    const ConvParams p = conv_desc_wdec_gemm(B, g, d.Cs_in, d.N);
    const int need = 26 + 7 * 9 + 8;
    if (cap < need) return fail(nullptr, VSTAB_E_NOMEM, "wdec_plan: need %d ints", need);
    put_desc(p, (int)TILE_128x128, 1, dec_layer(l), pl.wdec[l], out);
    const int gg[8] = {g.NTy, g.NTx, g.nty[0], g.nty[1], g.nty[2], g.ntx[0], g.ntx[1], g.ntx[2]};
    for (int i = 0; i < 8; ++i) out[26 + 63 + i] = gg[i];
    return need;
}

extern "C" long long vstab_host_pack_wdec(int l, const float *W, const double *scale, float *wpk, long long cap)
{
    if (!W || !wpk || l < 0 || l > 3) return fail(nullptr, VSTAB_E_SHAPE, "pack_wdec: bad arguments");
    const Layer &d = dec_layer(l);
    const int co = d.cout, cs = in_buf(d).cs;
    const long long n = 9LL * klayout_run(1, 1, cs).ktiles() * 4 * co * 32;
    if (cap < n) return fail(nullptr, VSTAB_E_NOMEM, "pack_wdec: need %lld floats", n);
    std::vector<double> ones;
    if (!scale) { ones.assign(co, 1.0); scale = ones.data(); }
    pack_wdec(W, scale, d.cin, cs, co, wpk);
    return n;
}

extern "C" long long vstab_host_pack_layer(int Cin, int layer, const float *W, const double *scale, float *wpk,
                                           long long cap)
{
    if (!W || !wpk || layer < 0 || layer > 18 || Cin < 1) return fail(nullptr, VSTAB_E_SHAPE, "pack_layer: bad arguments");
    std::vector<double> ones;
    const Layer &L = NET[layer];
    const int cs_in = layer == 0 ? Cin : in_buf(L).cs, npad = padded_cols(L.cout);
    if (L.kind == L_CONV) {
        const int ci = layer == 0 ? Cin : L.cin;
        const KLayout K = conv_layout(L.k, L.k, ci, cs_in);
        const long long n = (long long)K.ktiles() * npad * 32;
        if (cap < n) return fail(nullptr, VSTAB_E_NOMEM, "pack_layer: need %lld floats", n);
        if (!scale) { ones.assign(npad, 1.0); scale = ones.data(); }
        pack_conv(W, scale, L.k, L.k, ci, cs_in, L.cout, npad, K, wpk);
        return n;
    }
    if (L.kind == L_DECONV) {
        const long long n = 4LL * klayout_deconv(cs_in).ktiles() * npad * 32;
        if (cap < n) return fail(nullptr, VSTAB_E_NOMEM, "pack_layer: need %lld floats", n);
        if (!scale) { ones.assign(npad, 1.0); scale = ones.data(); }
        pack_deconv(W, scale, L.cin, cs_in, L.cout, npad, wpk);
        return n;
    }
    const long long n = (long long)klayout_run(1, 1, cs_in).ktiles() * 32 * 32;
    if (cap < n) return fail(nullptr, VSTAB_E_NOMEM, "pack_layer: need %lld floats", n);
    pack_predict2_table(W, L.cin, cs_in, 32, wpk);
    return n;
}
```

### coupe/optical_flow_based_deep_video_stabilization_amd/csrc/flownet_plan.h

```cpp
#pragma once
#include "api_internal.h"
#include "conv_desc.h"

enum Buf { B_CONV1, B_CONCAT2, B_CONV3, B_CONCAT3, B_CONV4, B_CONCAT4, B_CONV5, B_CONCAT5, B_CONV6, B_CONV6_1, B_T,
           B_T6, B_T5, B_T4, B_T3, B_TICKETS, B_PARTIAL, B_WINO_V, B_WINO_M, N_BUF };
static_assert(B_PARTIAL == N_BUF - 3 && B_WINO_V == N_BUF - 2 && B_WINO_M == N_BUF - 1, "plan-dependent buffers must come last");

struct BufSpec { const char *name; int level, c, cs; };
constexpr BufSpec BUFS[N_BUF] = {
    {"conv1", 0, 64, 64},         {"concat2", 1, 194, 196},   {"conv3", 2, 256, 256},     {"concat3", 3, 386, 388},
    {"conv4", 4, 512, 512},       {"concat4", 5, 770, 772},   {"conv5", 6, 512, 512},     {"concat5", 7, 1026, 1028},
    {"conv6", 8, 1024, 1024},     {"conv6_1", 9, 1024, 1024}, {"pf2_taps", 1, 32, 32},    {"pf6_taps", 9, 32, 32},
    {"pf5_taps", 7, 32, 32},      {"pf4_taps", 5, 32, 32},    {"pf3_taps", 3, 32, 32},    {"tickets", -1, 0, 0},
    {"splitk", -1, 0, 0},         {"winograd_in", -1, 0, 0},  {"winograd_out", -1, 0, 0}};

enum LayerKind { L_CONV, L_DECONV, L_TAPS };
struct Layer { const char *name; LayerKind kind; int k, s, p, cin, cout, in, out, c_off; };
constexpr int N_LAYER = 19;
constexpr Layer NET[N_LAYER] = {
    {"conv1", L_CONV, 7, 2, 3, 0, 64, -1, B_CONV1, 0},              {"conv2", L_CONV, 5, 2, 2, 64, 128, B_CONV1, B_CONCAT2, 0},
    {"conv3", L_CONV, 5, 2, 2, 128, 256, B_CONCAT2, B_CONV3, 0},    {"conv3_1", L_CONV, 3, 1, 1, 256, 256, B_CONV3, B_CONCAT3, 0},
    {"conv4", L_CONV, 3, 2, 1, 256, 512, B_CONCAT3, B_CONV4, 0},    {"conv4_1", L_CONV, 3, 1, 1, 512, 512, B_CONV4, B_CONCAT4, 0},
    {"conv5", L_CONV, 3, 2, 1, 512, 512, B_CONCAT4, B_CONV5, 0},    {"conv5_1", L_CONV, 3, 1, 1, 512, 512, B_CONV5, B_CONCAT5, 0},
    {"conv6", L_CONV, 3, 2, 1, 512, 1024, B_CONCAT5, B_CONV6, 0},   {"conv6_1", L_CONV, 3, 1, 1, 1024, 1024, B_CONV6, B_CONV6_1, 0},
    {"deconv5", L_DECONV, 4, 2, 1, 1024, 512, B_CONV6_1, B_CONCAT5, 512}, {"deconv4", L_DECONV, 4, 2, 1, 1026, 256, B_CONCAT5, B_CONCAT4, 512},
    {"deconv3", L_DECONV, 4, 2, 1, 770, 128, B_CONCAT4, B_CONCAT3, 256},  {"deconv2", L_DECONV, 4, 2, 1, 386, 64, B_CONCAT3, B_CONCAT2, 128},
    {"predict2", L_TAPS, 3, 1, 1, 194, 2, B_CONCAT2, B_T, 0},       {"predict6", L_TAPS, 3, 1, 1, 1024, 2, B_CONV6_1, B_T6, 0},
    {"predict5", L_TAPS, 3, 1, 1, 1026, 2, B_CONCAT5, B_T5, 0},     {"predict4", L_TAPS, 3, 1, 1, 770, 2, B_CONCAT4, B_T4, 0},
    {"predict3", L_TAPS, 3, 1, 1, 386, 2, B_CONCAT3, B_T3, 0}};
constexpr int LVL_ENC[5] = {9, 7, 5, 3, 1};
constexpr const Layer &dec_layer(int l) { return NET[10 + l]; }
constexpr const Layer &head_layer(int l) { return NET[15 + l]; }
constexpr const BufSpec &in_buf(const Layer &L) { return BUFS[L.in]; }
constexpr const BufSpec &out_buf(const Layer &L) { return BUFS[L.out]; }

constexpr bool net_is_consistent()
{
    for (int i = 1; i < 10; ++i)
        if (NET[i].in != NET[i - 1].out || NET[i].cin != NET[i - 1].cout || NET[i].cout > out_buf(NET[i]).c) return false;
    for (int i = 10; i < N_LAYER; ++i)
        if (NET[i].cin != in_buf(NET[i]).c) return false;
    for (int l = 0; l < 4; ++l) {
        const Layer &d = dec_layer(l);
        if (d.c_off + d.cout + 2 != out_buf(d).c || head_layer(l).in != d.in) return false;
        if (BUFS[d.out].level != LVL_ENC[l + 1] || BUFS[d.in].level != LVL_ENC[l] || BUFS[head_layer(l).out].level != LVL_ENC[l]) return false;
    }
    for (int b = 0; b < N_BUF; ++b)
        if (BUFS[b].cs < BUFS[b].c || (BUFS[b].cs & 3)) return false;
    return NET[14].in == dec_layer(3).out;
}
static_assert(net_is_consistent(), "NET and BUFS disagree");

struct Plan {
    int B, H, W, Cin;
    int eh[10], ew[10];
    size_t off[N_BUF];
    size_t bytes[N_BUF];
    size_t total;
    vstab::ConvParams cp[N_LAYER];
    vstab::ConvTile tile[N_LAYER];
    bool vec4[N_LAYER];
    bool conv1_bf16x3;
    bool skinny[N_LAYER];
    bool wino[10];
    vstab::ConvParams wcp[10];
    vstab::ConvTile wtile[10];
    bool wdec[4];
    vstab::ConvParams wdcp[4];
    vstab::ConvTile wdtile[4];
    vstab::WdecGeom wdg[4];
    int buf_h(int b) const { return BUFS[b].level < 0 ? 0 : eh[BUFS[b].level]; }
    int buf_w(int b) const { return BUFS[b].level < 0 ? 0 : ew[BUFS[b].level]; }
};

struct PlanPin { int batch = 0; unsigned flags = 0; };
inline PlanPin pin_of(const vstab_ctx *ctx)
{
    PlanPin pin;
    if (ctx) { pin.batch = ctx->plan_batch; pin.flags = ctx->plan_flags; }
    return pin;
}

bool level_sizes(int H, int W, int *eh, int *ew);
bool make_plan(int B, int H, int W, int Cin, Plan &pl, const PlanPin *pin = nullptr);
int chunk_size(const PlanPin &pin, int B, int H, int W, int Cin);
```

### coupe/optical_flow_based_deep_video_stabilization_amd/csrc/rowwin_tile.h

```cpp
#pragma once
#include <hip/hip_ext.h>

#include "vstab_internal.h"

namespace vstab {

typedef float f32x4 __attribute__((ext_vector_type(4)));
typedef float f32x16 __attribute__((ext_vector_type(16)));

typedef void (*RowWinKernel)(const RowWinParams);

constexpr unsigned ROWWIN_OOB = 0xC0000000u;

template <int MB>
struct RowWinTile {
    int tid, wm, wn, li, lh;
    int row, ox0, n;
    int pix_step, row_floats;
    int g0;
    __amdgpu_buffer_rsrc_t rin;
};

template <int MB>
__device__ __forceinline__ RowWinTile<MB> rowwin_tile(const RowWinParams &p)
{
    RowWinTile<MB> t;
    t.tid = threadIdx.x;
    const int lane = t.tid & 63, wave = t.tid >> 6;
    t.wm = wave >> 1; t.wn = wave & 1;
    t.li = lane & 31; t.lh = lane >> 5;
    unsigned bx_, by_, bz_;
    xcd_remap(bx_, by_, bz_);
    if (p.clear_n > 0 && blockIdx.x == 0 && blockIdx.y == 0 && blockIdx.z == 0)
        for (int i = t.tid; i < p.clear_n; i += 256) p.clear_words[i] = 0u;
    t.row = (int)bx_;
    t.ox0 = p.ox_base + (int)by_ * (64 * MB); t.n = (int)bz_;
    t.pix_step = p.s_in * p.Cs_in;
    t.row_floats = p.Wi * p.Cs_in;
    t.g0 = t.pix_step * t.ox0 + p.e_off - p.w_a;
    t.rin = __builtin_amdgcn_make_buffer_rsrc(const_cast<float *>(p.in), 0, p.in_bytes, 0x00020000);
    return t;
}

template <int MB>
__device__ __forceinline__ bool rowwin_chunk(const RowWinTile<MB> &t, const RowWinParams &p, int j, int &g)
{
    const int c4 = t.tid + 256 * j;
    g = t.g0 + 4 * c4;
    return g >= 0 && g < t.row_floats && 4 * c4 < p.WLEN;
}

template <int NWIN4, int MB>
__device__ __forceinline__ void rowwin_load_window(const RowWinTile<MB> &t, const RowWinParams &p, int oy, int ky, f32x4 (&wv)[NWIN4])
{
    const int iy = oy * p.s_in + p.off_y + ky;
    const bool yok = (unsigned)iy < (unsigned)p.Hi;
    const int rowbase = ((t.n * p.Hi + iy) * p.Wi) * p.Cs_in;
#pragma unroll
    for (int j = 0; j < NWIN4; ++j) {
        int g;
        const bool ok = rowwin_chunk(t, p, j, g) && yok;
        const unsigned off = ok ? (unsigned)(rowbase + g) * 4u : ROWWIN_OOB;
        wv[j] = __builtin_bit_cast(f32x4, __builtin_amdgcn_raw_buffer_load_b128(t.rin, off, 0, 0));
    }
}

template <int MB>
__device__ __forceinline__ int rowwin_acc_pixel(const RowWinTile<MB> &t, int mb, int r)
{
    return t.wm * 32 * MB + mb * 32 + (r & 3) + 8 * (r >> 2) + 4 * t.lh;
}

template <int MB>
__device__ __forceinline__ void rowwin_epilogue(const RowWinTile<MB> &t, const RowWinParams &p, const f32x16 (&acc)[MB], int oy, float *sC)
{
    const int col = t.wn * 32 + t.li;
    if (p.out_vec4) {
        constexpr int TP = 64 * MB;
        __syncthreads();
        const float bv = col < p.N ? p.bias[col] : 0.f;
#pragma unroll
        for (int mb = 0; mb < MB; ++mb)
#pragma unroll
            for (int r = 0; r < 16; ++r) sC[rowwin_acc_pixel(t, mb, r) * 64 + col] = acc[mb][r] + bv;
        __syncthreads();
        const float slope = p.act == 1 ? 0.1f : 0.0f;
        float *orow = p.out + ((long long)(t.n * p.Ho + oy) * p.Wo + t.ox0) * p.Cs_out + p.c_off;
#pragma unroll 4
        for (int e = t.tid; e < TP * 16; e += 256) {
            const int px = e >> 4, c4 = (e & 15) * 4;
            if (t.ox0 + px >= p.Wo || c4 >= p.N) continue;
            f32x4 v = *reinterpret_cast<const f32x4 *>(sC + px * 64 + c4);
            if (p.act) {
#pragma unroll
                for (int i = 0; i < 4; ++i) v[i] = fmaxf(v[i], slope * v[i]);
            }
            float *o = orow + (long long)px * p.Cs_out + c4;
            if (c4 + 4 <= p.N) *reinterpret_cast<f32x4 *>(o) = v;
            else for (int i = 0; c4 + i < p.N; ++i) o[i] = v[i];
        }
    } else if (col < p.N) {
        const float bv = p.bias[col];
#pragma unroll
        for (int mb = 0; mb < MB; ++mb)
#pragma unroll
            for (int r = 0; r < 16; ++r) {
                const int ox = t.ox0 + rowwin_acc_pixel(t, mb, r);
                if (ox < p.Wo) {
                    float v = acc[mb][r] + bv;
                    if (p.act) v = fmaxf(v, (p.act == 1 ? 0.1f : 0.0f) * v);
                    p.out[((long long)(t.n * p.Ho + oy) * p.Wo + ox) * p.Cs_out + p.c_off + col] = v;
                }
            }
    }
}

inline int rowwin_xtiles(const RowWinParams &p)
{
    const int tile = 64 * p.MB;
    if (p.ox_base < 0 || p.ox_base >= p.Wo || (p.ox_base & 1) || p.ntile_x < 0) return -1;
    return p.ntile_x > 0 ? p.ntile_x : (p.Wo - p.ox_base + tile - 1) / tile;
}

inline hipError_t rowwin_launch(RowWinParams q, RowWinKernel k72, RowWinKernel k41, size_t lds, hipStream_t stream, hipEvent_t ev_start,
                                hipEvent_t ev_stop)
{
    const int ntx = rowwin_xtiles(q);
    if (ntx < 0 || ((uintptr_t)q.in & 15) != 0) return hipErrorInvalidValue;
    dim3 grid(q.stream_rows > 0 ? q.Ho / q.stream_rows : q.Ho, ntx, q.B), block(256);
    q.out_vec4 = (((uintptr_t)q.out & 15) == 0 && (q.Cs_out & 3) == 0 && (q.c_off & 3) == 0 && lds >= (size_t)64 * q.MB * 64 * 4) ? 1 : 0;
    const RowWinKernel k = q.MB == 2 ? k72 : k41;
    if (ev_start || ev_stop) hipExtLaunchKernelGGL(k, grid, block, lds, stream, ev_start, ev_stop, 0, q);
    else k<<<grid, block, lds, stream>>>(q);
    return hipGetLastError();
}

inline hipError_t rowwin_set_lds_limits(RowWinKernel k72, int bytes72, RowWinKernel k41, int bytes41)
{
    const hipError_t e = hipFuncSetAttribute(reinterpret_cast<const void *>(k72), hipFuncAttributeMaxDynamicSharedMemorySize, bytes72);
    if (e != hipSuccess) return e;
    return hipFuncSetAttribute(reinterpret_cast<const void *>(k41), hipFuncAttributeMaxDynamicSharedMemorySize, bytes41);
}

}
```

### coupe/optical_flow_based_deep_video_stabilization_amd/csrc/vstab_internal.h

```cpp
#pragma once
#include <hip/hip_runtime.h>
#include <stddef.h>
#include <stdint.h>

namespace vstab {

inline int round_up_c(int a, int b) { return (a + b - 1) / b * b; }

#ifdef __HIPCC__
#define VSTAB_HD __host__ __device__
#else
#define VSTAB_HD
#endif
VSTAB_HD inline void xcd_remap_calc(unsigned Nx, unsigned Ny, unsigned Nz, unsigned lin, unsigned &bx, unsigned &by, unsigned &bz)
{
    const unsigned T = Nx * Ny * Nz;
    const unsigned q = T >> 3, r = T & 7u, c = lin & 7u, idx = lin >> 3;
    const unsigned nl = (c < r ? c * (q + 1) : r * (q + 1) + (c - r) * q) + idx;
    unsigned t2;
    if ((Ny & (Ny - 1)) == 0) { const unsigned s = 31u - (unsigned)__builtin_clz(Ny); by = nl & (Ny - 1); t2 = nl >> s; }
    else { by = nl % Ny; t2 = nl / Ny; }
    if ((Nz & (Nz - 1)) == 0) { const unsigned s = 31u - (unsigned)__builtin_clz(Nz); bz = t2 & (Nz - 1); bx = t2 >> s; }
    else { bz = t2 % Nz; bx = t2 / Nz; }
}
#ifdef __HIPCC__
__device__ __forceinline__ void xcd_remap(unsigned &bx, unsigned &by, unsigned &bz, bool identity = false)
{
    if (identity) { bx = blockIdx.x; by = blockIdx.y; bz = blockIdx.z; return; }
    xcd_remap_calc(gridDim.x, gridDim.y, gridDim.z, blockIdx.x + gridDim.x * (blockIdx.y + gridDim.y * blockIdx.z), bx, by, bz);
}
#endif

struct ConvPhase {
    int Hg, Wg, M;
    int off_y, off_x;
    int o_y, o_x;
    int pad_;
    long long w_off;
    int KH, NSEG, SEG, SEGP, SEG_STRIDE;
    int pad2_;
};

struct ConvParams {
    const float *in;
    const float *wpk;
    const float *bias;
    float *out;
    float *partial;
    unsigned in_bytes;
    unsigned w_bytes;
    int B, Hi, Wi, Cs_in;
    int KH;
    int NSEG, SEG, SEGP;
    int SEG_STRIDE;
    int s_in, s_out;
    int Ho, Wo, Cs_out, c_off;
    int N, Npad;
    int act;
    int nphase, ksplit, Mmax;
    int no_remap;
    int stamp_slot;
    int out_vec4;
    ConvPhase ph[16];
};

#ifdef __HIPCC__
__device__ __forceinline__ void splitk_combine_item(const ConvParams &p, const long long idx)
{
    typedef float f32x4 __attribute__((ext_vector_type(4)));

    const int n4 = p.N >> 2;
    const long long per_phase = (long long)p.Mmax * n4;
    if (idx >= per_phase * p.nphase) return;
    const int phase = (int)(idx / per_phase);
    const long long rem = idx - phase * per_phase;
    const int m = (int)(rem / n4), c4 = (int)(rem - (long long)m * n4);
    const ConvPhase ph = p.ph[phase];
    if (m >= ph.M) return;
    f32x4 s = {0.f, 0.f, 0.f, 0.f};
    const float *src = p.partial + (((long long)(phase * p.ksplit) * p.Mmax + m) * p.Npad + c4 * 4);
    const long long slab = (long long)p.Mmax * p.Npad;
    int k = 0;
    for (; k + 8 <= p.ksplit; k += 8) {
        f32x4 v[8];
#pragma unroll
        for (int u = 0; u < 8; ++u) v[u] = *reinterpret_cast<const f32x4 *>(src + (k + u) * slab);
#pragma unroll
        for (int u = 0; u < 8; ++u) s += v[u];
    }
    if (k + 4 <= p.ksplit) {
        f32x4 v[4];
#pragma unroll
        for (int u = 0; u < 4; ++u) v[u] = *reinterpret_cast<const f32x4 *>(src + (k + u) * slab);
#pragma unroll
        for (int u = 0; u < 4; ++u) s += v[u];
        k += 4;
    }
    if (k < p.ksplit) {
        f32x4 v[3];
#pragma unroll
        for (int u = 0; u < 3; ++u) v[u] = k + u < p.ksplit ? *reinterpret_cast<const f32x4 *>(src + (k + u) * slab) : f32x4{0.f, 0.f, 0.f, 0.f};
#pragma unroll
        for (int u = 0; u < 3; ++u)
            if (k + u < p.ksplit) s += v[u];
    }
    const f32x4 bv = *reinterpret_cast<const f32x4 *>(p.bias + c4 * 4);
    s += bv;
    if (p.act == 1 || p.act == 2) {
        const float slope = p.act == 1 ? 0.1f : 0.0f;
#pragma unroll
        for (int e = 0; e < 4; ++e) s[e] = fmaxf(s[e], slope * s[e]);
    }
    const int hw = ph.Hg * ph.Wg;
    const int n = m / hw, r2 = m - n * hw;
    const int j = r2 / ph.Wg, i = r2 - j * ph.Wg;
    const long long oo = ((long long)(n * p.Ho + j * p.s_out + ph.o_y) * p.Wo + i * p.s_out + ph.o_x) * p.Cs_out + p.c_off;
    if (p.act == 3) s += *reinterpret_cast<const f32x4 *>(p.out + oo + c4 * 4);
    *reinterpret_cast<f32x4 *>(p.out + oo + c4 * 4) = s;
}
#endif

enum ConvTile { TILE_128x128 = 0, TILE_128x64 = 1, TILE_128x32 = 2, TILE_64x128 = 3, TILE_64x64 = 4, TILE_256x32 = 5,
                TILE_SKINNY = 6 };

hipError_t launch_conv(const ConvParams &p, ConvTile tile, bool vec4, hipStream_t stream,
                       hipEvent_t ev_start = nullptr, hipEvent_t ev_stop = nullptr, bool combine = true);
hipError_t launch_conv_dual(const ConvParams &pa, ConvTile tile_a, const ConvParams &pb, ConvTile tile_b, hipStream_t stream,
                            hipEvent_t ev_start = nullptr, hipEvent_t ev_stop = nullptr);
hipError_t conv_set_attributes();
bool conv_uses_lds_dma(ConvTile tile, bool vec4);

constexpr int SKINNY_MAX_ROWS = 64;
constexpr int SKINNY_MAX_TILES = 4096;
bool conv_skinny_applicable(const ConvParams &p, bool vec4);
long long skinny_tiles(const ConvParams &p);
int conv_skinny_split(const ConvParams &p, int cap = 16);
hipError_t launch_conv_skinny(const ConvParams &p, unsigned *counters, hipStream_t stream, hipEvent_t ev_start = nullptr,
                              hipEvent_t ev_stop = nullptr);

struct RowWinParams {
    const float *in;
    const float *wpk;
    const float *bias;
    float *out;
    unsigned in_bytes;
    int B, Hi, Wi, Cs_in;
    int KH, SEGP;
    int s_in, off_y;
    int e_off;
    int w_a;
    int WLEN;
    int Ho, Wo, Cs_out, c_off;
    int N, Npad, act;
    int MB;
    int out_vec4;
    int asm_loop;
    int stream_rows;
    unsigned *clear_words;
    int clear_n;
    int ox_base, ntile_x;
};
inline int rowwin_mb(int B, int Ho, int Wo) { return (long long)B * Ho * ((Wo + 127) / 128) < 512 ? 1 : 2; }
inline bool rowwin_geometry_ok(const RowWinParams &p)
{
    return ((p.s_in * p.Cs_in) % 2 == 0) && ((p.Wi * p.Cs_in) % 4 == 0) && p.N <= 64 && p.Npad == 64 && (p.MB == 1 || p.MB == 2) &&
           p.WLEN <= (p.MB == 2 ? 7 : 4) * 1024 && (p.WLEN % 4) == 0 && p.in_bytes < 0x80000000u;
}
hipError_t rowwin_set_attributes();
hipError_t launch_conv_rowwin(const RowWinParams &p, hipStream_t stream, hipEvent_t ev_start = nullptr,
                              hipEvent_t ev_stop = nullptr);
inline int rowwin_lead(int off_x, int cs) { return ((off_x * cs) % 2 != 0) ? 1 : 0; }
inline int rowwin_segp(int off_x, int kw, int cs) { return round_up_c(rowwin_lead(off_x, cs) + kw * cs, 32); }
void pack_conv_rowwin(const float *W, const double *scale, int kh, int kw, int cin, int cout, int npad,
                      int lead, int segp, float *wpk);

inline bool conv1_bf16x3_geometry_ok(const RowWinParams &p) { return rowwin_geometry_ok(p) && p.KH >= 1 && (p.SEGP % 32) == 0 && p.SEGP >= 32; }
hipError_t conv1_bf16x3_set_attributes();
hipError_t launch_conv1_bf16x3(const RowWinParams &p, hipStream_t stream, hipEvent_t ev_start = nullptr,
                               hipEvent_t ev_stop = nullptr);
void pack_conv1_bf16x3(const float *W, const double *scale, int kh, int kw, int cin, int cout, int lead, int segp, uint16_t *wpk);

hipError_t launch_wino_outgrad(const float *dy, int B, int H, int W, int Cs, int c_off, int C, float *dM, hipStream_t stream);
hipError_t launch_wino_filter_grad(const float *dU, int cin, int cout, float *dW, hipStream_t stream);
int wino_gemm_stream_positions(int B, int T, int cin, int cout);
hipError_t launch_wino_gemm_stream(const float *V, const float *wpk, float *M, int B, int T, int cin, int cout, int P, hipStream_t stream,
                                   hipEvent_t ev_start = nullptr, hipEvent_t ev_stop = nullptr);
hipError_t wino_gemm_stream_set_attributes();
hipError_t launch_wino_input(const float *x, int B, int H, int W, int Cs, int c_off, int C, float *V, hipStream_t stream,
                             bool pos_major = false);
hipError_t launch_wino_weights(const float *W, int cin, int cout, int transpose, float *Wt, hipStream_t stream);
hipError_t launch_wino_output(const float *M, int B, int Ho, int Wo, int C, const float *bias, int act, float *out, int Cs_out, int c_off,
                              hipStream_t stream);

struct WdecGeom {
    int NTy, NTx;
    int nty[3], ntx[3];
};
inline WdecGeom wdec_geom(int Hi, int Wi, int Ho, int Wo)
{
    WdecGeom g;
    g.NTy = Ho / 4 + 1; g.NTx = Wo / 4 + 1;
    g.nty[0] = g.NTy < Hi / 2 + 1 ? g.NTy : Hi / 2 + 1; g.nty[1] = g.nty[2] = g.NTy < (Hi + 1) / 2 ? g.NTy : (Hi + 1) / 2;
    g.ntx[0] = g.NTx < Wi / 2 + 1 ? g.NTx : Wi / 2 + 1; g.ntx[1] = g.ntx[2] = g.NTx < (Wi + 1) / 2 ? g.NTx : (Wi + 1) / 2;
    return g;
}
struct WdecOutArgs { const float *M; int C4; const float *bias; int act; float *out; int Ho, Wo, Cs_out, c_off; WdecGeom g; };
#ifdef __HIPCC__
__device__ __forceinline__ void wdec_output_item(const WdecOutArgs &A, const long long idx, const int n)
{
    typedef float f32x4 __attribute__((ext_vector_type(4)));
    const WdecGeom &g = A.g;
    const int C4 = A.C4;
    if (idx >= (long long)g.NTy * g.NTx * 4 * C4) return;
    const int c = (int)(idx % C4);
    const int ph = (int)((idx / C4) & 3);
    const int tile = (int)(idx / (4 * C4));
    const int ty = tile / g.NTx, tx = tile - ty * g.NTx;
    const int py = ph >> 1, px = ph & 1;
    const int N = 16 * C4;
    const long long plane = (long long)g.NTy * g.NTx * N;
    const float *mb = A.M + (long long)n * 9 * plane + (long long)tile * N + ph * (4 * C4) + c * 4;
    f32x4 m[3][3];
#pragma unroll
    for (int i = 0; i < 3; ++i)
#pragma unroll
        for (int j = 0; j < 3; ++j) {
            f32x4 v = {0.f, 0.f, 0.f, 0.f};
            if (ty < g.nty[i] && tx < g.ntx[j]) v = *reinterpret_cast<const f32x4 *>(mb + (i * 3 + j) * plane);
            m[i][j] = v;
        }
    f32x4 s[2][3];
#pragma unroll
    for (int j = 0; j < 3; ++j) {
        s[0][j] = m[0][j] + m[1][j];
        s[1][j] = m[1][j] - m[2][j];
    }
    const f32x4 bv = *reinterpret_cast<const f32x4 *>(A.bias + c * 4);
    const float slope = A.act == 1 ? 0.1f : 0.0f;
#pragma unroll
    for (int a = 0; a < 2; ++a) {
        const int oy = 4 * ty + 2 * a - py;
        if ((unsigned)oy >= (unsigned)A.Ho) continue;
#pragma unroll
        for (int b = 0; b < 2; ++b) {
            const int ox = 4 * tx + 2 * b - px;
            if ((unsigned)ox >= (unsigned)A.Wo) continue;
            f32x4 y = (b == 0 ? s[a][0] + s[a][1] : s[a][1] - s[a][2]) + bv;
            if (A.act) {
#pragma unroll
                for (int e = 0; e < 4; ++e) y[e] = fmaxf(y[e], slope * y[e]);
            }
            *reinterpret_cast<f32x4 *>(A.out + (((long long)n * A.Ho + oy) * A.Wo + ox) * A.Cs_out + A.c_off + c * 4) = y;
        }
    }
}
#endif
hipError_t launch_wdec_input(const float *x, int B, int Hi, int Wi, int Cs, float *V, const WdecGeom &g, hipStream_t stream);
hipError_t launch_wdec_output(const float *M, int B, int Ho, int Wo, int cout, const float *bias, int act, float *out, int Cs_out, int c_off,
                              const WdecGeom &g, hipStream_t stream);

struct UpflowW { float w[64]; float b[2]; };
hipError_t launch_predict_up(const float *src, int ks, long long slab_stride, int B, int h, int w, const float *bias2,
                             const float *prev, int ph, int pw, float *out, const UpflowW &W, float *concat, int oh, int ow,
                             int Cs, int c_off, hipStream_t stream, const ConvParams *combine = nullptr, const WdecOutArgs *wdec = nullptr);

bool tap_panel_applicable(long long M, int cs_in, const void *x, const void *T);
hipError_t launch_tap_panel(const float *x, long long M, const float *wp, float *T, hipStream_t stream, hipEvent_t ev_start = nullptr,
                            hipEvent_t ev_stop = nullptr);
hipError_t tap_panel_set_attributes();
hipError_t launch_pf2(const float *T, int B, int h2, int w2, const float *bias2, const float *pf3,
                      int h3, int w3, float *pf2, int H, int W, hipStream_t stream);

hipError_t launch_flow_resize_scale(const float *flow, int B, int h, int w, float *out, int oh,
                                    int ow, int net_h, int net_w, hipStream_t stream);
hipError_t launch_resize_bilinear(const float *x, int B, int h, int w, int C, float *out, int oh,
                                  int ow, hipStream_t stream);
hipError_t launch_resize_bilinear_slice3(const float *x, int B, int h, int w, int Cs, int c_off, float *out, int oh, int ow,
                                         hipStream_t stream);
hipError_t launch_warp_flow(const float *img, const float *flow, float *out, int B, int H, int W,
                            int C, hipStream_t stream);
enum { HBM_SLOT_WARP = 0, HBM_SLOT_GLUE = 1, HBM_SLOT_GLUE_WARP = 2, HBM_SLOT_PF2 = 3, HBM_SLOT_ST = 4, HBM_SLOT_HOMOG = 5, HBM_SLOT_TAIL = 6, HBM_SLOTS = 7 };
void hbm_profile_enable(int mode);
hipError_t hbm_profile_read(int slot, double *ms_sum, int *launches, double *alg_bytes_sum);
hipError_t launch_div_const_selftest(float d, unsigned first, unsigned long long count, unsigned long long *bad, hipStream_t stream);
hipError_t launch_pf2_glue_warp(const float *T, int B, int h2, int w2, const float *bias2, const float *pf3, int h3, int w3, float *pf2, int H, int W,
                                const float *img, float *outflow, float *out, int oh, int ow, hipStream_t stream);
hipError_t launch_pf2_glue_warp_u8(const float *T, int B, int h2, int w2, const float *bias2, const float *pf3, int h3, int w3, float *pf2, int H, int W,
                                   const unsigned char *frame, float *outflow, unsigned char *out, int oh, int ow, hipStream_t stream);
hipError_t launch_flow_glue_warp(const float *flow, int B, int h, int w, const float *img, float *outflow, float *out, int oh, int ow,
                                 int C, int net_h, int net_w, hipStream_t stream);
hipError_t launch_maxpool2x2(const float *x, int B, int H, int W, int C, float *out, hipStream_t stream);
hipError_t launch_conv3x3_rgb(const float *x, int B, int H, int W, const float *Wf, const float *bias, int cout, int relu, float *out,
                              hipStream_t stream);
hipError_t launch_scale_shift(const float *x, long long npix, int C, float scale, const float *mean4, float *out,
                              hipStream_t stream);
hipError_t launch_get_pixel_value(const float *img, const int32_t *x, const int32_t *y, float *out,
                                  int B, int H, int W, int C, int Hi, int Wi, hipStream_t stream);

hipError_t launch_st_interp(const float *img, int B, int H, int W, int C, const float *x, const float *y,
                            int oh, int ow, float *out, hipStream_t stream);
hipError_t launch_st_transform(const float *img, int B, int H, int W, int C, const float *theta, int tdim,
                               float *out, int oh, int ow, hipStream_t stream);
hipError_t launch_st_meshgrid(float *out, int oh, int ow, hipStream_t stream);
hipError_t launch_homography_warp(const float *img, int B, int Hi, int Wi, int C, const float *M, float *out,
                                  int oh, int ow, hipStream_t stream, const float *ref = nullptr);
hipError_t launch_vec2mtrx(const float *p, int B, int dim, int approx, float *out, hipStream_t stream);
hipError_t launch_st_bicubic_interp(const float *img, int B, int H, int W, int C, const float *x, const float *y, int oh, int ow,
                                    float *out, hipStream_t stream);
hipError_t launch_st_transform_interp(const float *img, int B, int H, int W, int C, const float *theta, int tdim, int interp,
                                      float *out, int oh, int ow, hipStream_t stream);
hipError_t launch_st_symmetry_transform(const float *img, int B, int H, int W, int C, const float *theta, int kind, int interp,
                                        float *out, int oh, int ow, hipStream_t stream);
hipError_t launch_st_elastic_transform(const float *img, int B, int H, int W, int C, const float *theta, int g, const float *linv_t,
                                       int interp, float *out, int oh, int ow, hipStream_t stream);
size_t st_transform_backward_ws_bytes(int B, int H, int W, int C, int oh, int ow);
hipError_t launch_st_transform_backward(const float *img, int B, int H, int W, int C, const float *theta, int tdim, const float *dout, int oh,
                                        int ow, float *d_img, int accumulate, float *d_theta, double *part, hipStream_t stream);
hipError_t launch_st_interp_backward(const float *img, int B, int H, int W, int C, const float *x, const float *y, const float *dout, int oh,
                                     int ow, float *d_img, int accumulate, float *d_x, float *d_y, hipStream_t stream);
hipError_t launch_st_elastic_coords(const float *theta, int B, int g, const float *linv_t, int oh, int ow, float *x_out, float *y_out,
                                    hipStream_t stream);
size_t st_elastic_backward_ws_bytes(int B, int H, int W, int C, int g, int oh, int ow);
hipError_t launch_st_elastic_transform_backward(const float *img, int B, int H, int W, int C, const float *theta, int g, const float *linv_t,
                                                const float *dout, int oh, int ow, float *d_img, int accumulate, float *d_theta, double *part,
                                                hipStream_t stream);

bool st3d_plan(int B, int od, int oh, int ow, int &nbx, int &nby, int &nbz, long long &bricks);
hipError_t launch_st3d_meshgrid(float *out, int od, int oh, int ow, hipStream_t stream);
hipError_t launch_st3d_interp(const float *vol, int B, int D, int H, int W, int C, const float *x, const float *y, const float *z, int od, int oh,
                              int ow, int edge, float *out, hipStream_t stream);
hipError_t launch_st3d_transform(const float *vol, int B, int D, int H, int W, int C, const float *theta, float *out, int od, int oh, int ow,
                                 hipStream_t stream);
size_t st3d_transform_backward_ws_bytes(int B, int od, int oh, int ow);
hipError_t launch_st3d_transform_backward(const float *vol, int B, int D, int H, int W, int C, const float *theta, const float *dout, int od, int oh,
                                          int ow, float *d_vol, int accumulate, float *d_theta, double *part, hipStream_t stream);
hipError_t launch_st3d_interp_backward(const float *vol, int B, int D, int H, int W, int C, const float *x, const float *y, const float *z,
                                       int od, int oh, int ow, int edge, const float *dout, float *d_vol, int accumulate, float *d_x, float *d_y,
                                       float *d_z, hipStream_t stream);

hipError_t launch_resize_u8(const unsigned char *src, int B, int sh, int sw, unsigned char *dst, int dh, int dw, hipStream_t stream);
hipError_t launch_resize_f32_to_u8(const float *src, int B, int sh, int sw, unsigned char *dst, int dh, int dw, hipStream_t stream);
hipError_t launch_assemble_input(const unsigned char *const *slots9, int B, int h, int w, float *feats, hipStream_t stream);
hipError_t launch_assemble_input_resized(const unsigned char *const *slots8, const unsigned char *frame, int B, int h, int w, int sh, int sw,
                                         float *feats, hipStream_t stream);
hipError_t launch_flow_glue_warp_u8(const float *flow, int B, int h, int w, const unsigned char *frame, float *outflow, unsigned char *out, int oh,
                                    int ow, int net_h, int net_w, hipStream_t stream);
hipError_t launch_frame_to_float(const unsigned char *f, long long npix, float *out, hipStream_t stream);
hipError_t launch_quantise_output(const float *warped, long long npix, unsigned char *out, hipStream_t stream);

hipError_t launch_flow_box_blur(const float *flow, int B, int h, int w, int k, float *tmp, float *out, hipStream_t stream);
hipError_t launch_axpby(const float *x, float a, const float *y, float b, float *out, long long n, hipStream_t stream);
hipError_t launch_flow_mean_fill(const float *flow, int B, int h, int w, float *out, hipStream_t stream);
struct WgradParams {
    const float *x;
    const float *g;
    const int4 *ptab;
    float *dW;
    float *partial;
    unsigned x_bytes, g_bytes;
    int Hi, Wi, Cs_x, cx_off, Cin;
    int KH, KW;
    int Cs_g, cg_off, Cout;
    int M, K;
    int ksplit, accumulate;
    int nbatch;
    long long x_bstride, g_bstride;
    int ldw, col0;
};
hipError_t launch_wgrad_pixel_table(int B, int Hi, int Wi, int Cs, int Ho, int Wo, int s, int pad, int4 *ptab, hipStream_t stream);
int wgrad_choose_split(const WgradParams &p);
hipError_t launch_wgrad(const WgradParams &p, hipStream_t stream);
inline int reduce_chunks(long long rows, int C)
{
    const long long colblocks = C >= 64 ? (C + 63) / 64 : 1;
    long long n = 768 / colblocks;
    if (n < 8) n = 8;
    const long long by_rows = rows / 128;
    if (n > by_rows) n = by_rows;
    return (int)(n < 1 ? 1 : n);
}
int column_sum_chunks(long long rows, int C);
hipError_t launch_column_sum(const float *g, long long rows, int Cs, int c_off, int C, float *out, int accumulate, float *scratch,
                             hipStream_t stream);

hipError_t launch_loss_level(const float *pf, const float *G, const float *U, int B, int h, int w, double *sums, float scale_mse,
                             float scale_tv, float *grad, hipStream_t stream);
struct LossLevel { const float *pf; float *grad; int h, w, cs_pf, cs_grad; float tv_weight; };
size_t loss_main_workspace_bytes(int B, const LossLevel *lv, int n);
hipError_t launch_loss_main(const LossLevel *lv, int n, const float *gtstab, const float *unstab, int B, int H, int W, double *loss_out,
                            void *workspace, hipStream_t stream);
hipError_t launch_flow_medfilt(const float *flow, int B, int h, int w, int kh, int kw, int kc, float *out, hipStream_t stream);

int homography_moment_blocks(int H, int W);
size_t homography_workspace_bytes(int B, int H, int W, int K);
hipError_t launch_homography_fit(const float *flow, int B, int H, int W, int K, unsigned seed, double thresh, int refine,
                                 int stride, double *Hout, int *inliers, void *ws, hipStream_t stream);
hipError_t launch_warp_perspective_u8(const unsigned char *src, int B, int sh, int sw, const double *Hm, unsigned char *dst,
                                      int oh, int ow, hipStream_t stream);

hipError_t launch_contrast(float *buf, int B, int H, int W, int C, int Cs, int c_dst, hipStream_t stream);
hipError_t launch_nldf_score(const float *local2, const float *global2, int B, int npix, float *score, float *prob,
                             hipStream_t stream);

inline int round_up(int a, int b) { return (a + b - 1) / b * b; }

inline int swz32(int n, int k) { return ((((k >> 2) ^ ((n >> 1) & 7)) << 2) | (k & 3)); }

struct KLayout {
    int KH, NSEG, SEG, SEGP, SEG_STRIDE;
    int ktiles() const { return KH * NSEG * (SEGP / 32); }
};
KLayout klayout_run(int kh, int kw, int cs_in);
KLayout klayout_tap(int kh, int kw, int cin, int cs_in);

void fold_bn(const float *b, const float *beta, const float *mean, const float *var, int cout,
             int npad, double *scale, float *bias_out);

void pack_conv(const float *W, const double *scale, int kh, int kw, int cin, int cs_in, int cout,
               int npad, const KLayout &L, float *wpk);

void pack_deconv(const float *W, const double *scale, int cin, int cs_in, int cout, int npad,
                 float *wpk);
KLayout klayout_deconv(int cs_in);

void pack_deconv5(const float *W, const double *scale, int cin, int cs_in, int cout, int npad, float *wpk);

void pack_winograd(const float *W, const double *scale, int cin, int cout, int npad, float *wpk);

void pack_wdec(const float *W, const double *scale, int cin, int cs_in, int cout, float *wpk);

void pack_predict2_table(const float *W, int cin, int cs_in, int npad, float *wpk);
void pack_predict2_panel(const float *W, int cin, int kpad, float *wp);

int bn_chunks(long long rows, int C);
hipError_t launch_bn_lrelu_train_forward(float *zy, long long rows, int cs, int c_off, int C, const float *beta, float *mov_mean,
                                         float *mov_var, float decay, float eps, float *save_mean, float *save_rstd, float *scratch,
                                         hipStream_t stream);
hipError_t launch_bn_lrelu_train_backward(const float *y, int cs_y, int cy_off, float *dy, int cs_g, int cg_off, int C, long long rows,
                                          const float *beta, const float *save_rstd, float *dbeta, int accumulate, float *scratch,
                                          hipStream_t stream);
hipError_t launch_lrelu_backward(const float *y, int cs_y, int cy_off, float *dy, int cs_g, int cg_off, int C, long long rows,
                                 hipStream_t stream);

hipError_t launch_resize_bilinear_backward(const float *dout, int B, int oh, int ow, int C, float *din, int h, int w, float gain,
                                           int accumulate, hipStream_t stream);
hipError_t launch_pad_nearest_up(const float *src, int B, int h2, int w2, int C, float *out, int H, int W, hipStream_t stream);
hipError_t launch_pad_nearest_up_backward(const float *dout, int B, int H, int W, int C, float *dsrc, int h2, int w2, int accumulate,
                                          hipStream_t stream);
hipError_t launch_pf2_taps_backward(const float *g, int cs_g, int B, int H, int W, float *dT, int h2, int w2, hipStream_t stream);
hipError_t launch_adam(float *w, const float *g, float *m, float *v, long long n, float lr_t, float b1, float b2, float eps,
                       hipStream_t stream);

void pack_index_conv(int kh, int kw, int cin, int cs_in, int cout, int npad, const KLayout &L, int32_t *tbl);
void pack_index_dgrad_s1(int k, int cin, int cout, int cs_g, const KLayout &L, int npad, int32_t *tbl);
void pack_index_dgrad_s2(int k, int pad, int cin, int cout, int cs_g, const KLayout &L, int npad, int32_t *tbl);
void pack_index_phase(int k, int cin, int cout, int cs_g, const KLayout &L, int npad, int t0y, int nty, int t0x, int ntx, int32_t *tbl);
hipError_t launch_pack_apply(const float *W, const int32_t *tbl, long long n, float *wpk, hipStream_t stream, bool n_fast = false);
hipError_t launch_pack_blocked(const float *W, int K, int N, int Npad, int batch, float *wpk, hipStream_t stream);

}
```

### include/vstab.h

```cpp
#ifndef VSTAB_H
#define VSTAB_H

#include <stddef.h>
#include <stdint.h>

#ifdef __cplusplus
extern "C" {
#endif

#define VSTAB_OK          0
#define VSTAB_E_SHAPE    -1
#define VSTAB_E_ALIGN    -2
#define VSTAB_E_HIP      -3
#define VSTAB_E_NOMEM    -4
#define VSTAB_E_WEIGHTS  -5
#define VSTAB_E_STATE    -6

#if defined(__GNUC__)
#define VSTAB_API __attribute__((visibility("default")))
#else
#define VSTAB_API
#endif

typedef struct vstab_ctx vstab_ctx;

typedef struct vstab_tensor {
    const char  *name;
    const float *data;
    int32_t      ndim;
    int32_t      shape[4];
} vstab_tensor;

typedef struct vstab_ws_entry {
    char    name[24];
    int64_t offset_bytes;
    int32_t n, h, w, c;
    int32_t c_stride;
} vstab_ws_entry;

VSTAB_API int  vstab_create(vstab_ctx **out, int device);
VSTAB_API void vstab_destroy(vstab_ctx *ctx);
VSTAB_API const char *vstab_last_error(const vstab_ctx *ctx);
VSTAB_API const char *vstab_version(void);

VSTAB_API int vstab_load_weights(vstab_ctx *ctx, const vstab_tensor *tensors, int count);

VSTAB_API size_t vstab_workspace_bytes(int B, int H, int W, int Cin);

VSTAB_API int vstab_set_plan_batch(vstab_ctx *ctx, int batch);
VSTAB_API size_t vstab_workspace_bytes_ctx(const vstab_ctx *ctx, int B, int H, int W, int Cin);

VSTAB_API int vstab_workspace_layout(int B, int H, int W, int Cin, vstab_ws_entry *entries, int max_entries);
VSTAB_API int vstab_workspace_layout_ctx(const vstab_ctx *ctx, int B, int H, int W, int Cin, vstab_ws_entry *entries, int max_entries);

VSTAB_API int vstab_flownets_forward(vstab_ctx *ctx, const float *feats, int B, int H, int W, int Cin,
                           float *pf6, float *pf5, float *pf4, float *pf3, float *pf2,
                           void *workspace, size_t workspace_bytes, void *stream);

VSTAB_API int vstab_flow_resize_scale(const float *flow, int B, int h, int w, float *out, int oh, int ow,
                            int net_h, int net_w, void *stream);

VSTAB_API int vstab_resize_bilinear(const float *x, int B, int h, int w, int C, float *out, int oh, int ow,
                          void *stream);

VSTAB_API int vstab_resize_bilinear_slice3(const float *x, int B, int h, int w, int Cs, int c_off, float *out, int oh, int ow,
                                 void *stream);

VSTAB_API int vstab_warp_flow(const float *img, const float *flow, float *out, int B, int H, int W, int C,
                    void *stream);

VSTAB_API int vstab_flow_glue_warp(const float *flow, int B, int h, int w, const float *img, float *outflow, float *warped,
                         int oh, int ow, int C, int net_h, int net_w, void *stream);

VSTAB_API int vstab_stabilise_originalsize(vstab_ctx *ctx, const float *feats, int B, int H, int W, int Cin, const float *frame,
                                           int oh, int ow, float *pf6, float *pf5, float *pf4, float *pf3, float *pf2,
                                           float *outflow, float *warped, void *workspace, size_t workspace_bytes, void *stream);

VSTAB_API int vstab_get_pixel_value(const float *img, const int32_t *x, const int32_t *y, float *out, int B,
                          int H, int W, int C, int Hi, int Wi, void *stream);

VSTAB_API int vstab_st_transform(const float *img, int B, int H, int W, int C, const float *theta, int theta_dim,
                                 float *out, int oh, int ow, void *stream);
VSTAB_API int vstab_st_bilinear_interp(const float *img, int B, int H, int W, int C, const float *x, const float *y,
                                       int oh, int ow, float *out, void *stream);
VSTAB_API int vstab_st_meshgrid(float *out, int oh, int ow, void *stream);
#define VSTAB_INTERP_BILINEAR 0
#define VSTAB_INTERP_BICUBIC  1
#define VSTAB_SYM_AFFINE      0
#define VSTAB_SYM_PROJECTIVE  1
#define VSTAB_SYM_SIMILARITY  2
#define VSTAB_TPS_GMAX       16
VSTAB_API int vstab_st_bicubic_interp(const float *img, int B, int H, int W, int C, const float *x, const float *y, int oh, int ow,
                                      float *out, void *stream);
VSTAB_API int vstab_st_transform_interp(const float *img, int B, int H, int W, int C, const float *theta, int theta_dim, int interp,
                                        float *out, int oh, int ow, void *stream);
VSTAB_API int vstab_st_symmetry_transform(const float *img, int B, int H, int W, int C, const float *theta, int kind, int interp,
                                          float *out, int oh, int ow, void *stream);
VSTAB_API int vstab_host_tps_linv(int g, float *linv_t, int cap);
VSTAB_API int vstab_st_elastic_transform(const float *img, int B, int H, int W, int C, const float *theta, int g, const float *linv_t,
                                         int interp, float *out, int oh, int ow, void *stream);
VSTAB_API size_t vstab_st_transform_backward_workspace_bytes(int B, int H, int W, int C, int oh, int ow);
VSTAB_API int vstab_st_transform_backward(const float *img, int B, int H, int W, int C, const float *theta, int theta_dim,
                                          const float *dout, int oh, int ow, float *d_img, int accumulate, float *d_theta,
                                          void *workspace, size_t workspace_bytes, void *stream);
VSTAB_API int vstab_st_bilinear_interp_backward(const float *img, int B, int H, int W, int C, const float *x, const float *y,
                                                const float *dout, int oh, int ow, float *d_img, int accumulate, float *d_x,
                                                float *d_y, void *stream);
VSTAB_API int vstab_st_elastic_coords(const float *theta, int B, int g, const float *linv_t, int oh, int ow, float *x_out, float *y_out,
                                      void *stream);
VSTAB_API size_t vstab_st_elastic_transform_backward_workspace_bytes(int B, int H, int W, int C, int g, int oh, int ow);
VSTAB_API int vstab_st_elastic_transform_backward(const float *img, int B, int H, int W, int C, const float *theta, int g,
                                                  const float *linv_t, const float *dout, int oh, int ow, float *d_img, int accumulate,
                                                  float *d_theta, void *workspace, size_t workspace_bytes, void *stream);
#ifndef VSTAB_ST3D_BRICK_Z
#define VSTAB_ST3D_BRICK_Z 2
#define VSTAB_ST3D_BRICK_Y 8
#define VSTAB_ST3D_BRICK_X 16
#endif
VSTAB_API int vstab_st3d_meshgrid(float *out, int od, int oh, int ow, void *stream);
VSTAB_API int vstab_st3d_bilinear_interp(const float *vol, int B, int D, int H, int W, int C, const float *x, const float *y,
                                         const float *z, int od, int oh, int ow, int edge_size, float *out, void *stream);
VSTAB_API int vstab_st3d_transform(const float *vol, int B, int D, int H, int W, int C, const float *theta, float *out, int od,
                                   int oh, int ow, void *stream);
VSTAB_API size_t vstab_st3d_transform_backward_workspace_bytes(int B, int D, int H, int W, int C, int od, int oh, int ow);
VSTAB_API int vstab_st3d_transform_backward(const float *vol, int B, int D, int H, int W, int C, const float *theta, const float *dout,
                                            int od, int oh, int ow, float *d_vol, int accumulate, float *d_theta, void *workspace,
                                            size_t workspace_bytes, void *stream);
VSTAB_API int vstab_st3d_bilinear_interp_backward(const float *vol, int B, int D, int H, int W, int C, const float *x, const float *y,
                                                  const float *z, int od, int oh, int ow, int edge_size, const float *dout,
                                                  float *d_vol, int accumulate, float *dx, float *dy, float *dz, void *stream);
VSTAB_API int vstab_homography_warp(const float *img, int B, int Hi, int Wi, int C, const float *M, float *out, int oh,
                                    int ow, void *stream);
VSTAB_API int vstab_transform_image(const float *img, int B, int Hi, int Wi, int C, const float *ref, const float *pM, float *out,
                                    int oh, int ow, void *stream);
VSTAB_API int vstab_vec2mtrx(const float *p, int B, int dim, int warp_approx, float *out, void *stream);

VSTAB_API int vstab_vgg16_load(vstab_ctx *ctx, const vstab_tensor *tensors, int count);
VSTAB_API size_t vstab_vgg16_workspace_bytes(int B, int H, int W);
VSTAB_API int vstab_vgg16_shapes(int H, int W, int32_t *hwc54);
VSTAB_API int vstab_vgg16_forward(vstab_ctx *ctx, const float *input, int B, int H, int W, float *const *outputs18,
                                  void *workspace, size_t workspace_bytes, void *stream);
VSTAB_API int vstab_scale_shift(const float *x, long long npix, int C, float scale, const float *mean, float *out,
                                void *stream);
VSTAB_API int vstab_maxpool2x2(const float *x, int B, int H, int W, int C, float *out, void *stream);

VSTAB_API int vstab_nldf_load(vstab_ctx *ctx, const vstab_tensor *tensors, int count);
VSTAB_API size_t vstab_nldf_workspace_bytes(int B);
VSTAB_API int vstab_nldf_forward(vstab_ctx *ctx, const float *const *pools5, int B, float *prob, float *score,
                                 float *local_fea, float *fea_global, void *workspace, size_t workspace_bytes,
                                 void *stream);

VSTAB_API int vstab_resize_u8(const uint8_t *src, int B, int sh, int sw, uint8_t *dst, int dh, int dw, void *stream);
VSTAB_API int vstab_resize_f32_to_u8(const float *src, int B, int sh, int sw, uint8_t *dst, int dh, int dw, void *stream);
VSTAB_API int vstab_assemble_input(const uint8_t *const *slots9, int B, int h, int w, float *feats, void *stream);
VSTAB_API int vstab_assemble_input_resized(const uint8_t *const *slots8, const uint8_t *frame, int B, int h, int w, int sh, int sw,
                                           float *feats, void *stream);
VSTAB_API int vstab_flow_glue_warp_u8(const float *flow, int B, int h, int w, const uint8_t *frame, float *outflow, uint8_t *out, int oh, int ow,
                                      int net_h, int net_w, void *stream);
VSTAB_API int vstab_clip_step(vstab_ctx *ctx, const uint8_t *const *slots8, const uint8_t *frame, int n, int net_h, int net_w, int oh, int ow,
                              float *feats, float *pf6, float *pf5, float *pf4, float *pf3, float *pf2, float *outflow, uint8_t *out,
                              uint8_t *ring_slot, void *workspace, size_t workspace_bytes, void *stream);
VSTAB_API int vstab_frame_to_float(const uint8_t *frame, long long npix, float *out, void *stream);
VSTAB_API int vstab_quantise_output(const float *warped, long long npix, uint8_t *out, void *stream);

VSTAB_API int vstab_flow_box_blur(const float *flow, int B, int h, int w, int k, float *tmp, float *out, void *stream);
VSTAB_API int vstab_axpby(const float *x, float a, const float *y, float b, float *out, long long n, void *stream);
VSTAB_API int vstab_loss_level(const float *pf, const float *gt, const float *unstab, int B, int h, int w, double *sums,
                               float scale_mse, float scale_tv, float *grad_pf, void *stream);

typedef struct vstab_loss_level_desc {
    const float *pf;
    float *grad;
    int h, w, cs_pf, cs_grad;
    float tv_weight;
} vstab_loss_level_desc;
VSTAB_API size_t vstab_loss_main_workspace_bytes(const vstab_loss_level_desc *levels, int n_levels, int B);
VSTAB_API int vstab_loss_main(const vstab_loss_level_desc *levels, int n_levels, const float *gtstab, const float *unstab, int B, int H,
                              int W, double *loss_out, void *workspace, size_t workspace_bytes, void *stream);

VSTAB_API size_t vstab_conv_wgrad_workspace_bytes(int B, int Ho, int Wo, int k, int cin, int cout);
VSTAB_API int vstab_conv_wgrad(const float *x, int B, int Hi, int Wi, int cs_x, int cx_off, int cin, const float *gout, int Ho,
                               int Wo, int cs_g, int cg_off, int cout, int k, int stride, int pad, float *dW, float *db,
                               int accumulate, void *workspace, size_t workspace_bytes, void *stream);

VSTAB_API size_t vstab_conv_dgrad_workspace_bytes(int B, int Ho, int Wo, int cs_g, int cout, int k, int stride, int pad, int Hi, int Wi,
                                                  int cs_x, int cx_off, int cin, int accumulate);
VSTAB_API int vstab_conv_dgrad(const float *gout, int B, int Ho, int Wo, int cs_g, int cg_off, int cout, const float *W,
                               const float *bias , int k, int stride, int pad,
                               float *dx, int Hi, int Wi, int cs_x, int cx_off, int cin, int accumulate, void *workspace,
                               size_t workspace_bytes, void *stream);
VSTAB_API size_t vstab_conv_forward_workspace_bytes(int B, int Hi, int Wi, int cs_x, int cin, int k, int stride, int pad, int cout, int cs_y,
                                                    int cy_off, int act, int Ho, int Wo);
VSTAB_API int vstab_conv_forward(const float *x, int B, int Hi, int Wi, int cs_x, int cx_off, int cin, const float *W, const float *bias,
                                 int k, int stride, int pad, float *y, int Ho, int Wo, int cs_y, int cy_off, int cout, int act,
                                 void *workspace, size_t workspace_bytes, void *stream);
VSTAB_API size_t vstab_conv_rowwin_forward_workspace_bytes(int B, int H, int W, int Cin, int cs_w, int cout, int k, int stride, int pad, int cs_y,
                                                           int cy_off, int act);
VSTAB_API int vstab_conv_rowwin_forward(const float *x, int B, int H, int W, int Cin, const float *Wf, int cs_w, int cout, const float *bias, int k,
                                        int stride, int pad, float *y, int cs_y, int cy_off, int act, void *workspace, size_t workspace_bytes,
                                        void *stream);
VSTAB_API size_t vstab_conv3x3_winograd_workspace_bytes(int B, int H, int W, int cin, int cout, int transpose);
VSTAB_API int vstab_conv3x3_winograd(const float *x, int B, int H, int W, int cs_x, int cx_off, const float *Wf, int cin, int cout, int transpose,
                                     const float *bias, float *y, int cs_y, int cy_off, int act, void *workspace, size_t workspace_bytes,
                                     void *stream);
VSTAB_API size_t vstab_conv3x3_winograd_wgrad_workspace_bytes(int B, int H, int W, int cin, int cout);
VSTAB_API int vstab_conv3x3_winograd_wgrad(const float *x, int B, int H, int W, int cs_x, int cx_off, int cin, const float *gout, int cs_g,
                                           int cg_off, int cout, float *dW, void *workspace, size_t workspace_bytes, void *stream);
VSTAB_API int vstab_resize_bilinear_backward(const float *dout, int B, int oh, int ow, int C, float *din, int h, int w, float gain,
                                             int accumulate, void *stream);
VSTAB_API int vstab_pad_nearest_upsample(const float *src, int B, int h2, int w2, int C, float *out, int H, int W, void *stream);
VSTAB_API int vstab_pad_nearest_upsample_backward(const float *dout, int B, int H, int W, int C, float *dsrc, int h2, int w2, int accumulate,
                                                  void *stream);
VSTAB_API int vstab_pf2_from_taps(const float *T, int B, int h2, int w2, const float *bias2, const float *pf3, int h3, int w3, float *pf2,
                                  int H, int W, void *stream);
VSTAB_API int vstab_pf2_taps_backward(const float *g, int cs_g, int B, int H, int W, float *dT, int h2, int w2, void *stream);
VSTAB_API int vstab_predict2_tap_table(const float *concat2, long long M, const float *table, float *T, void *stream);
VSTAB_API size_t vstab_column_sum_scratch_bytes(long long rows, int C);
VSTAB_API int vstab_column_sum(const float *g, long long rows, int cs, int c_off, int C, float *out, int accumulate, void *scratch,
                               size_t scratch_bytes, void *stream);
VSTAB_API int vstab_adam_step(float *w, const float *g, float *m, float *v, long long n, float lr_t, float beta1, float beta2, float eps,
                              void *stream);

VSTAB_API size_t vstab_bn_scratch_bytes(long long rows, int C);
VSTAB_API int vstab_bn_lrelu_train_forward(float *zy, long long rows, int cs, int c_off, int C, const float *beta, float *moving_mean,
                                           float *moving_var, float decay, float eps, float *save_mean, float *save_rstd, void *scratch,
                                           size_t scratch_bytes, void *stream);
VSTAB_API int vstab_bn_lrelu_train_backward(const float *y, int cs_y, int cy_off, float *dy, int cs_g, int cg_off, int C, long long rows,
                                            const float *beta, const float *save_rstd, float *dbeta, int accumulate, void *scratch,
                                            size_t scratch_bytes, void *stream);
VSTAB_API int vstab_lrelu_backward(const float *y, int cs_y, int cy_off, float *dy, int cs_g, int cg_off, int C, long long rows, void *stream);

VSTAB_API int vstab_flow_medfilt(const float *flow, int B, int h, int w, int kh, int kw, int kc, float *out, void *stream);
VSTAB_API int vstab_flow_mean_fill(const float *flow, int B, int h, int w, float *out, void *stream);

VSTAB_API size_t vstab_homography_workspace_bytes(int B, int H, int W, int K);
VSTAB_API int vstab_homography_fit(const float *flow, int B, int H, int W, int K, unsigned seed, double thresh, int refine,
                                   int stride, double *Hout, int32_t *inliers, void *workspace, size_t workspace_bytes,
                                   void *stream);
VSTAB_API int vstab_warp_perspective_u8(const uint8_t *src, int B, int sh, int sw, const double *Hm, uint8_t *dst, int oh, int ow,
                                        void *stream);


#define VSTAB_PLAN_NO_SKINNY 1u
#define VSTAB_PLAN_NO_DUAL 2u
#define VSTAB_PLAN_NO_TAIL 4u
#define VSTAB_PLAN_NO_WDEC 8u
#define VSTAB_PLAN_FORCE_WDEC 16u
#define VSTAB_PLAN_CONV1_FP32 32u
VSTAB_API int vstab_set_plan_flags(vstab_ctx *ctx, unsigned flags);

VSTAB_API int vstab_conv1_forward(vstab_ctx *ctx, const float *feats, int B, int H, int W, int Cin, float *out, int cs_out, int c_off,
                                  void *stream);

VSTAB_API int vstab_profile_enable(vstab_ctx *ctx, int enable);
VSTAB_API int vstab_profile_reset(vstab_ctx *ctx);
VSTAB_API int vstab_profile_read(vstab_ctx *ctx, double *ms_sum15, double *flops15, int *n_forwards);
VSTAB_API int vstab_profile_read_direct(vstab_ctx *ctx, double *flops15);
VSTAB_API int vstab_profile_kernel_name(vstab_ctx *ctx, int slot, char *buf, int cap);

VSTAB_API int vstab_selftest_div_const(float d, unsigned first_bits, unsigned long long count, unsigned long long *bad_count_dev,
                                       void *stream);

VSTAB_API int vstab_trace_ranges(int on);

VSTAB_API int vstab_hbm_profile_enable(int mode);
VSTAB_API int vstab_hbm_profile_read(int slot, double *ms_sum, int *launches, double *alg_bytes_sum);

VSTAB_API int vstab_host_xcd_remap(int gx, int gy, int gz, int lin, int32_t *xyz);
VSTAB_API int vstab_level_sizes(int H, int W, int32_t *hw20);

VSTAB_API int vstab_host_layer_plan(int B, int H, int W, int Cin, int layer, int32_t *out, int cap);
VSTAB_API int vstab_host_layer_plan_pinned(int plan_batch, unsigned flags, int B, int H, int W, int Cin, int layer, int32_t *out, int cap);

VSTAB_API long long vstab_host_pack_layer(int Cin, int layer, const float *W, const double *scale,
                                          float *wpk, long long cap);

VSTAB_API int vstab_host_wdec_plan(int B, int H, int W, int Cin, int l, int32_t *out, int cap);
VSTAB_API long long vstab_host_pack_wdec(int l, const float *W, const double *scale, float *wpk, long long cap);

#ifdef __cplusplus
}
#endif
#endif
```

Before: 2996 frame-pairs/s.

## Compute two output rows per workgroup in bf16x3 conv1, sharing input windows

The bf16x3 conv1 kernel can now produce two adjacent output rows per workgroup. Each staged input row window is reused for both rows' MFMAs with different weight slices, so the input windows that the rows share are loaded and split once instead of twice. The bf16 split is also moved into registers and interleaved with the MFMA issue through sched_group_barrier, and weight loads use buffer loads. Two-row mode is chosen when there are enough workgroups, or when forced by a flag. It doubles the accumulator registers (launch_bounds min 2 blocks) and halves the grid size.

```diff
diff --git a/coupe/optical_flow_based_deep_video_stabilization_amd/csrc/conv1_bf16x3.hip b/coupe/optical_flow_based_deep_video_stabilization_amd/csrc/conv1_bf16x3.hip
--- a/coupe/optical_flow_based_deep_video_stabilization_amd/csrc/conv1_bf16x3.hip
+++ b/coupe/optical_flow_based_deep_video_stabilization_amd/csrc/conv1_bf16x3.hip
@@ -7,48 +7,56 @@
 typedef __bf16 bf16x4 __attribute__((ext_vector_type(4)));
 typedef __bf16 bf16x8 __attribute__((ext_vector_type(8)));
 
-template <int NWIN4, int MB>
-__global__ __launch_bounds__(256) void conv1_bf16x3_kernel(const RowWinParams p)
+template <int NWIN4, int MB, int ROWS>
+__global__ __launch_bounds__(256, 2) void conv1_bf16x3_kernel(const RowWinParams p)
 {
     extern __shared__ __attribute__((aligned(16))) char smem[];
     unsigned *planes = reinterpret_cast<unsigned *>(smem);
 
-    const RowWinTile<MB> t = rowwin_tile<MB>(p);
+    const RowWinTile<MB> t = rowwin_tile<MB>(p, ROWS);
     const int tid = t.tid, wm = t.wm, wn = t.wn, li = t.li, lh = t.lh;
     const int oy = t.row, pix_step = t.pix_step;
+    const bool two = ROWS == 2 && oy + 1 < p.Ho;
 
     f32x4 wv[NWIN4];
-    auto load_window = [&](int ky) { rowwin_load_window(t, p, oy, ky, wv); };
+    u32x2 pk[NWIN4][3];
+    auto load_window = [&](int j) __attribute__((always_inline)) { rowwin_load_window(t, p, oy, j, wv); };
+    auto split = [&](int j) __attribute__((always_inline)) {
+        if (j >= NWIN4) return;
+        bf16x4 h, m, l;
+#pragma unroll
+        for (int e = 0; e < 4; ++e) {
+            const float x = wv[j][e];
+            h[e] = (__bf16)x;
+            const float r1 = x - (float)h[e];
+            m[e] = (__bf16)r1;
+            const float r2 = r1 - (float)m[e];
+            l[e] = (__bf16)r2;
+        }
+        pk[j][0] = __builtin_bit_cast(u32x2, h);
+        pk[j][1] = __builtin_bit_cast(u32x2, m);
+        pk[j][2] = __builtin_bit_cast(u32x2, l);
+    };
     const int plane_w = p.WLEN >> 1;
-    auto split_store = [&]() {
+    auto store_planes = [&]() __attribute__((always_inline)) {
 #pragma unroll
         for (int j = 0; j < NWIN4; ++j) {
             const int c4 = tid + 256 * j;
             if (4 * c4 < p.WLEN) {
-                bf16x4 h, m, l;
-#pragma unroll
-                for (int e = 0; e < 4; ++e) {
-                    const float x = wv[j][e];
-                    h[e] = (__bf16)x;
-                    const float r1 = x - (float)h[e];
-                    m[e] = (__bf16)r1;
-                    const float r2 = r1 - (float)m[e];
-                    l[e] = (__bf16)r2;
-                }
-                *reinterpret_cast<u32x2 *>(planes + 2 * c4) = __builtin_bit_cast(u32x2, h);
-                *reinterpret_cast<u32x2 *>(planes + plane_w + 2 * c4) = __builtin_bit_cast(u32x2, m);
-                *reinterpret_cast<u32x2 *>(planes + 2 * plane_w + 2 * c4) = __builtin_bit_cast(u32x2, l);
+#pragma unroll
+                for (int q = 0; q < 3; ++q) *reinterpret_cast<u32x2 *>(planes + q * plane_w + 2 * c4) = pk[j][q];
             }
         }
     };
 
     const int KG = p.SEGP >> 4;
     const int NG = p.KH * KG;
-    const unsigned *bbase = reinterpret_cast<const unsigned *>(p.wpk) + (wn * 32 + li) * 8 + lh * 4;
-    auto load_b = [&](u32x4 (&b)[3], int G) {
-        const unsigned *s = bbase + (long long)(G < NG ? G : NG - 1) * (3 * 512);
-#pragma unroll
-        for (int q = 0; q < 3; ++q) b[q] = *reinterpret_cast<const u32x4 *>(s + q * 512);
+    const __amdgpu_buffer_rsrc_t rw = __builtin_amdgcn_make_buffer_rsrc(const_cast<float *>(p.wpk), 0, NG * (3 * 512 * 4), 0x00020000);
+    const int b_lane = ((wn * 32 + li) * 8 + lh * 4) * 4;
+    auto load_b = [&](u32x4 (&b)[3], int G) __attribute__((always_inline)) {
+        const int s = (G < NG ? G : NG - 1) * (3 * 512 * 4);
+#pragma unroll
+        for (int q = 0; q < 3; ++q) b[q] = __builtin_bit_cast(u32x4, __builtin_amdgcn_raw_buffer_load_b128(rw, b_lane, s + q * 2048, 0));
     };
     const int a_w0 = (pix_step * (wm * 32 * MB + li) + p.w_a + 8 * lh) >> 1;
     const int a_w1 = a_w0 + ((pix_step * 32) >> 1);
@@ -64,58 +72,124 @@
             }
     };
 
-    f32x16 acc[MB];
-#pragma unroll
-    for (int a = 0; a < MB; ++a)
-#pragma unroll
-        for (int r = 0; r < 16; ++r) acc[a][r] = 0.f;
-
-    auto mma = [&](const u32x4 (&a)[3 * MB], const u32x4 (&b)[3]) {
+    f32x16 acc[ROWS][MB];
+#pragma unroll
+    for (int r = 0; r < ROWS; ++r)
+#pragma unroll
+        for (int a = 0; a < MB; ++a)
+#pragma unroll
+            for (int i = 0; i < 16; ++i) acc[r][a][i] = 0.f;
+
+    auto mma = [&](f32x16 (&c)[MB], const u32x4 (&a)[3 * MB], const u32x4 (&b)[3]) {
         constexpr int PA[6] = {2, 1, 0, 1, 0, 0}, PB[6] = {0, 1, 2, 0, 1, 0};
 #pragma unroll
         for (int t = 0; t < 6; ++t)
 #pragma unroll
             for (int mb = 0; mb < MB; ++mb)
-                acc[mb] = __builtin_amdgcn_mfma_f32_32x32x16_bf16(__builtin_bit_cast(bf16x8, a[mb * 3 + PA[t]]),
-                                                                  __builtin_bit_cast(bf16x8, b[PB[t]]), acc[mb], 0, 0, 0);
+                c[mb] = __builtin_amdgcn_mfma_f32_32x32x16_bf16(__builtin_bit_cast(bf16x8, a[mb * 3 + PA[t]]),
+                                                                __builtin_bit_cast(bf16x8, b[PB[t]]), c[mb], 0, 0, 0);
+    };
+    auto mma_split = [&](f32x16 (&c)[MB], const u32x4 (&a)[3 * MB], const u32x4 (&b)[3], int chunk) {
+        split(chunk);
+        mma(c, a, b);
+#pragma unroll
+        for (int i = 0; i < 6 * MB; ++i) {
+            __builtin_amdgcn_sched_group_barrier(0x008, 1, 0);
+            __builtin_amdgcn_sched_group_barrier(0x002, 8 / MB, 0);
+        }
     };
 
     u32x4 a0[3 * MB], a1[3 * MB], b0[3], b1[3];
+    auto row_one = [&](f32x16 (&c)[MB], int Gs, int Gnext) {
+        int g = 0;
+        auto trip = [&](int c0) __attribute__((always_inline)) {
+            load_a(a1, g + 1);
+            load_b(b1, Gs + g + 1);
+            __builtin_amdgcn_sched_barrier(0);
+            mma_split(c, a0, b0, c0);
+            __builtin_amdgcn_sched_barrier(0);
+            if (g + 2 < KG) load_a(a0, g + 2);
+            load_b(b0, g + 2 < KG ? Gs + g + 2 : Gnext);
+            __builtin_amdgcn_sched_barrier(0);
+            mma_split(c, a1, b1, c0 + 1);
+            __builtin_amdgcn_sched_barrier(0);
+            g += 2;
+        };
+        trip(NWIN4);
+#pragma unroll
+        for (int c0 = 0; c0 < NWIN4; c0 += 2) {
+            if (g < KG) trip(c0);
+            else { split(c0); split(c0 + 1); }
+        }
+        while (g < KG) trip(NWIN4);
+    };
+    auto row_two = [&](int GA, int GB, int Gnext) __attribute__((always_inline)) {
+        int g = 0;
+        auto trip = [&](int c0) __attribute__((always_inline)) {
+            load_a(a1, g + 1);
+            load_b(b1, GB + g);
+            __builtin_amdgcn_sched_barrier(0);
+            mma_split(acc[0], a0, b0, c0);
+            __builtin_amdgcn_sched_barrier(0);
+            load_b(b0, GA + g + 1);
+            __builtin_amdgcn_sched_barrier(0);
+            mma(acc[ROWS - 1], a0, b1);
+            __builtin_amdgcn_sched_barrier(0);
+            if (g + 2 < KG) load_a(a0, g + 2);
+            load_b(b1, GB + g + 1);
+            __builtin_amdgcn_sched_barrier(0);
+            mma_split(acc[0], a1, b0, c0 + 1);
+            __builtin_amdgcn_sched_barrier(0);
+            load_b(b0, g + 2 < KG ? GA + g + 2 : Gnext);
+            __builtin_amdgcn_sched_barrier(0);
+            mma(acc[ROWS - 1], a1, b1);
+            __builtin_amdgcn_sched_barrier(0);
+            g += 2;
+        };
+        trip(NWIN4);
+#pragma unroll
+        for (int c0 = 0; c0 < NWIN4; c0 += 2) {
+            if (g < KG) trip(c0);
+            else { split(c0); split(c0 + 1); }
+        }
+        while (g < KG) trip(NWIN4);
+    };
+
+    const int NJ = two ? p.KH + p.s_in : p.KH;
     load_window(0);
     load_b(b0, 0);
-    split_store();
+#pragma unroll
+    for (int j = 0; j < NWIN4; ++j) split(j);
+    store_planes();
     __syncthreads();
-    int G = 0;
-    for (int ky = 0; ky < p.KH; ++ky) {
-        const bool more = ky + 1 < p.KH;
-        if (more) load_window(ky + 1);
+    auto staged = [&](int j, auto body) __attribute__((always_inline)) {
+        const bool more = j + 1 < NJ;
+        if (more) load_window(j + 1);
         load_a(a0, 0);
         __builtin_amdgcn_sched_barrier(0);
-        for (int g = 0; g < KG; g += 2, G += 2) {
-            load_a(a1, g + 1);
-            load_b(b1, G + 1);
-            __builtin_amdgcn_sched_barrier(0);
-            mma(a0, b0);
-            __builtin_amdgcn_sched_barrier(0);
-            if (g + 2 < KG) load_a(a0, g + 2);
-            load_b(b0, G + 2);
-            __builtin_amdgcn_sched_barrier(0);
-            mma(a1, b1);
-            __builtin_amdgcn_sched_barrier(0);
-        }
+        body((j + 1 < p.KH ? j + 1 : j + 1 - p.s_in) * KG);
         if (more) {
             __syncthreads();
-            split_store();
+            store_planes();
             __syncthreads();
         }
+    };
+    const int n_first = (ROWS == 2 && two) ? p.s_in : NJ;
+    for (int j = 0; j < n_first; ++j) staged(j, [&](int Gnext) __attribute__((always_inline)) { row_one(acc[0], j * KG, Gnext); });
+    if (ROWS == 2) {
+        for (int j = n_first; j < p.KH; ++j) staged(j, [&](int Gnext) __attribute__((always_inline)) { row_two(j * KG, (j - p.s_in) * KG, Gnext); });
+        for (int j = p.KH; j < NJ; ++j) staged(j, [&](int Gnext) __attribute__((always_inline)) { row_one(acc[ROWS - 1], (j - p.s_in) * KG, Gnext); });
     }
 
-    rowwin_epilogue(t, p, acc, oy, reinterpret_cast<float *>(smem));
+    rowwin_epilogue(t, p, acc[0], oy, reinterpret_cast<float *>(smem));
+    if (ROWS == 2 && two) rowwin_epilogue(t, p, acc[ROWS - 1], oy + 1, reinterpret_cast<float *>(smem));
 }
 
 hipError_t conv1_bf16x3_set_attributes()
 {
-    return rowwin_set_lds_limits(conv1_bf16x3_kernel<7, 2>, 3 * 7 * 1024 * 2, conv1_bf16x3_kernel<4, 1>, 3 * 4 * 1024 * 2);
+    const hipError_t e = rowwin_set_lds_limits(conv1_bf16x3_kernel<7, 2, 1>, 3 * 7 * 1024 * 2, conv1_bf16x3_kernel<4, 1, 1>, 3 * 4 * 1024 * 2);
+    if (e != hipSuccess) return e;
+    return rowwin_set_lds_limits(conv1_bf16x3_kernel<7, 2, 2>, 3 * 7 * 1024 * 2, conv1_bf16x3_kernel<4, 1, 2>, 3 * 4 * 1024 * 2);
 }
 
 hipError_t launch_conv1_bf16x3(const RowWinParams &p, hipStream_t stream, hipEvent_t ev_start, hipEvent_t ev_stop)
@@ -124,7 +198,9 @@
     RowWinParams q = p;
     q.asm_loop = 0;
     q.stream_rows = 0;
-    return rowwin_launch(q, conv1_bf16x3_kernel<7, 2>, conv1_bf16x3_kernel<4, 1>, (size_t)3 * p.WLEN * 2, stream, ev_start, ev_stop);
-}
-
-}
+    const size_t lds = (size_t)3 * p.WLEN * 2;
+    if (p.rows == 2) return rowwin_launch(q, conv1_bf16x3_kernel<7, 2, 2>, conv1_bf16x3_kernel<4, 1, 2>, lds, stream, ev_start, ev_stop);
+    return rowwin_launch(q, conv1_bf16x3_kernel<7, 2, 1>, conv1_bf16x3_kernel<4, 1, 1>, lds, stream, ev_start, ev_stop);
+}
+
+}
diff --git a/coupe/optical_flow_based_deep_video_stabilization_amd/csrc/conv_desc.cpp b/coupe/optical_flow_based_deep_video_stabilization_amd/csrc/conv_desc.cpp
--- a/coupe/optical_flow_based_deep_video_stabilization_amd/csrc/conv_desc.cpp
+++ b/coupe/optical_flow_based_deep_video_stabilization_amd/csrc/conv_desc.cpp
@@ -69,7 +69,7 @@
 }
 
 RowWinDesc rowwin_desc(int B, int H, int W, int cin, int k, int stride, int pad, int Ho, int Wo, int cout, int npad, int cs_out, int c_off,
-                       int act)
+                       int act, RowWinPair pair)
 {
     RowWinDesc d;
     std::memset(&d, 0, sizeof d);
@@ -83,6 +83,11 @@
     r.Ho = Ho; r.Wo = Wo; r.Cs_out = cs_out; r.c_off = c_off; r.N = cout; r.Npad = npad; r.act = act;
     auto tile = [](RowWinParams &q, int MB) { q.MB = MB; q.WLEN = round_up(q.s_in * q.Cs_in * (64 * MB - 1) + q.w_a + q.SEGP, 4); };
     tile(r, rowwin_mb(B, Ho, Wo));
+    {
+        const long long xtiles = (Wo + 64 * r.MB - 1) / (64 * r.MB), pairs = (long long)B * ((Ho + 1) / 2) * xtiles;
+        const bool fits = k > stride && stride >= 1;
+        r.rows = fits && (pair == ROWWIN_PAIR_FORCE || (pair == ROWWIN_PAIR_RULE && pairs >= ROWWIN_PAIR_MIN_WORKGROUPS)) ? 2 : 1;
+    }
     d.ok = rowwin_geometry_ok(r);
     const int rem = Wo % 128;
     if (d.ok && r.MB == 2 && Wo > 128 && rem >= 1 && rem <= 64) {
diff --git a/coupe/optical_flow_based_deep_video_stabilization_amd/csrc/conv_desc.h b/coupe/optical_flow_based_deep_video_stabilization_amd/csrc/conv_desc.h
--- a/coupe/optical_flow_based_deep_video_stabilization_amd/csrc/conv_desc.h
+++ b/coupe/optical_flow_based_deep_video_stabilization_amd/csrc/conv_desc.h
@@ -33,6 +33,7 @@
 vstab::ConvParams conv_desc_wino_gemm(int B, int H, int W, int cin, int cout);
 vstab::ConvParams conv_desc_wdec_gemm(int B, const vstab::WdecGeom &g, int cs_in, int cout);
 
+enum RowWinPair { ROWWIN_PAIR_NEVER = -1, ROWWIN_PAIR_RULE = 0, ROWWIN_PAIR_FORCE = 1 };
 struct RowWinDesc { vstab::RowWinParams main, tail; bool ok, two; };
 RowWinDesc rowwin_desc(int B, int H, int W, int cin, int k, int stride, int pad, int Ho, int Wo, int cout, int npad, int cs_out, int c_off,
-                       int act);
+                       int act, RowWinPair pair = ROWWIN_PAIR_NEVER);
diff --git a/coupe/optical_flow_based_deep_video_stabilization_amd/csrc/conv_rowwin.hip b/coupe/optical_flow_based_deep_video_stabilization_amd/csrc/conv_rowwin.hip
--- a/coupe/optical_flow_based_deep_video_stabilization_amd/csrc/conv_rowwin.hip
+++ b/coupe/optical_flow_based_deep_video_stabilization_amd/csrc/conv_rowwin.hip
@@ -200,6 +200,7 @@
     const int ntx = rowwin_xtiles(p);
     if (!rowwin_geometry_ok(p) || ntx < 0) return hipErrorInvalidValue;
     RowWinParams q = p;
+    q.rows = 1;
     q.asm_loop = ((p.SEGP >> 5) == 6 && p.KH >= 1 && 4 * p.WLEN <= (p.MB == 2 ? VSTAB_ROWWIN_BUF_BYTES : VSTAB_ROWWIN1_BUF_BYTES)) ? 1 : 0;
 #ifdef VSTAB_NO_ASM_KLOOP
     q.asm_loop = 0;
diff --git a/coupe/optical_flow_based_deep_video_stabilization_amd/csrc/flownet_forward.cpp b/coupe/optical_flow_based_deep_video_stabilization_amd/csrc/flownet_forward.cpp
--- a/coupe/optical_flow_based_deep_video_stabilization_amd/csrc/flownet_forward.cpp
+++ b/coupe/optical_flow_based_deep_video_stabilization_amd/csrc/flownet_forward.cpp
@@ -173,14 +173,14 @@
     return VSTAB_OK;
 }
 
-static int conv1_rowwin(vstab_ctx *ctx, bool bf16x3, const float *feats, int B, int H, int W, int Cin, int Ho, int Wo, int N, int Npad,
+static int conv1_rowwin(vstab_ctx *ctx, bool bf16x3, int pair, const float *feats, int B, int H, int W, int Cin, int Ho, int Wo, int N, int Npad,
                         float *out, int cs_out, int c_off, unsigned *tickets, hipStream_t stream, hipEvent_t ev_a, hipEvent_t ev_b,
                         const char **kname, bool *launched)
 {
     const Layer &e = NET[0];
     const float *dw = ctx->dev_weights;
     *launched = false;
-    RowWinDesc d = rowwin_desc(B, H, W, Cin, e.k, e.s, e.p, Ho, Wo, N, Npad, cs_out, c_off, 1);
+    RowWinDesc d = rowwin_desc(B, H, W, Cin, e.k, e.s, e.p, Ho, Wo, N, Npad, cs_out, c_off, 1, (RowWinPair)pair);
     if (!d.ok || ((uintptr_t)feats & 15) != 0) return VSTAB_OK;
     const bool b3 = bf16x3 && ctx->enc0_b3 != 0 && conv1_bf16x3_geometry_ok(d.main);
     RowWinParams &r = d.main, &t = d.tail;
@@ -194,11 +194,13 @@
     if (d.two) {
         HIP_TRY(ctx, launch1(r, ev_a, nullptr));
         HIP_TRY(ctx, launch1(t, nullptr, ev_b));
-        *kname = b3 ? "conv1_bf16x3_kernel<7, 2> + <4, 1> tail" : "conv_rowwin_kernel<7, 2> + <4, 1> tail";
+        if (b3) *kname = r.rows == 2 ? "conv1_bf16x3_kernel<7, 2, 2> + <4, 1, 2> tail" : "conv1_bf16x3_kernel<7, 2, 1> + <4, 1, 1> tail";
+        else *kname = "conv_rowwin_kernel<7, 2> + <4, 1> tail";
         return VSTAB_OK;
     }
     HIP_TRY(ctx, launch1(r, ev_a, ev_b));
-    if (b3) *kname = r.MB == 2 ? "conv1_bf16x3_kernel<7, 2>" : "conv1_bf16x3_kernel<4, 1>";
+    if (b3 && r.rows == 2) *kname = r.MB == 2 ? "conv1_bf16x3_kernel<7, 2, 2>" : "conv1_bf16x3_kernel<4, 1, 2>";
+    else if (b3) *kname = r.MB == 2 ? "conv1_bf16x3_kernel<7, 2, 1>" : "conv1_bf16x3_kernel<4, 1, 1>";
     else *kname = r.MB == 2 ? "conv_rowwin_kernel<7, 2>" : "conv_rowwin_kernel<4, 1>";
     return VSTAB_OK;
 }
@@ -220,7 +222,7 @@
     if (((uintptr_t)feats & 15) || ((uintptr_t)out & 3)) return fail(ctx, VSTAB_E_ALIGN, "conv1_forward: feats must be 16-byte aligned");
     const char *kname = nullptr;
     bool launched = false;
-    const int rc = conv1_rowwin(ctx, pl->conv1_bf16x3, feats, B, H, W, Cin, p.Ho, p.Wo, p.N, p.Npad, out, cs_out, c_off, nullptr,
+    const int rc = conv1_rowwin(ctx, pl->conv1_bf16x3, pl->conv1_pair, feats, B, H, W, Cin, p.Ho, p.Wo, p.N, p.Npad, out, cs_out, c_off, nullptr,
                                 (hipStream_t)stream_, nullptr, nullptr, &kname, &launched);
     if (rc != VSTAB_OK) return rc;
     if (!launched) return fail(ctx, VSTAB_E_SHAPE, "conv1_forward: the row-window kernels do not take this geometry");
@@ -286,7 +288,7 @@
         if (i == 0) {
             const char *kname = nullptr;
             bool launched = false;
-            const int rc = conv1_rowwin(ctx, pl.conv1_bf16x3, feats, B, H, W, Cin, p.Ho, p.Wo, p.N, p.Npad, buf(B_CONV1), p.Cs_out, 0,
+            const int rc = conv1_rowwin(ctx, pl.conv1_bf16x3, pl.conv1_pair, feats, B, H, W, Cin, p.Ho, p.Wo, p.N, p.Npad, buf(B_CONV1), p.Cs_out, 0,
                                         tickets_cleared ? nullptr : tickets, stream, EV_A(0), EV_B(0), &kname, &launched);
             if (rc != VSTAB_OK) return rc;
             if (launched) { tickets_cleared = true; PROF_NAME(0, kname); continue; }
diff --git a/coupe/optical_flow_based_deep_video_stabilization_amd/csrc/flownet_plan.cpp b/coupe/optical_flow_based_deep_video_stabilization_amd/csrc/flownet_plan.cpp
--- a/coupe/optical_flow_based_deep_video_stabilization_amd/csrc/flownet_plan.cpp
+++ b/coupe/optical_flow_based_deep_video_stabilization_amd/csrc/flownet_plan.cpp
@@ -193,6 +193,7 @@
     }
     pl.conv1_bf16x3 = ref ? ref->conv1_bf16x3
                           : (!(flags & VSTAB_PLAN_CONV1_FP32) && NET[0].cout == 64 && rowwin_segp(-NET[0].p, NET[0].k, Cin) <= 192);
+    pl.conv1_pair = (flags & VSTAB_PLAN_CONV1_ONE_ROW) ? ROWWIN_PAIR_NEVER : ((flags & VSTAB_PLAN_CONV1_FORCE_PAIR) ? ROWWIN_PAIR_FORCE : ROWWIN_PAIR_RULE);
     size_t wino_v = 0, wino_m = 0;
     for (int i = 0; i < 10; ++i) {
         pl.wino[i] = false;
@@ -310,7 +311,11 @@
 extern "C" int vstab_set_plan_flags(vstab_ctx *ctx, unsigned flags)
 {
     if (!ctx) return fail(nullptr, VSTAB_E_STATE, "set_plan_flags: ctx is NULL");
-    if (flags & ~(unsigned)(VSTAB_PLAN_NO_SKINNY | VSTAB_PLAN_NO_DUAL | VSTAB_PLAN_NO_TAIL | VSTAB_PLAN_NO_WDEC | VSTAB_PLAN_FORCE_WDEC | VSTAB_PLAN_CONV1_FP32)) return fail(ctx, VSTAB_E_SHAPE, "set_plan_flags: unknown flag bits 0x%x", flags);
+    if (flags & ~(unsigned)(VSTAB_PLAN_NO_SKINNY | VSTAB_PLAN_NO_DUAL | VSTAB_PLAN_NO_TAIL | VSTAB_PLAN_NO_WDEC | VSTAB_PLAN_FORCE_WDEC | VSTAB_PLAN_CONV1_FP32 |
+                            VSTAB_PLAN_CONV1_ONE_ROW | VSTAB_PLAN_CONV1_FORCE_PAIR))
+        return fail(ctx, VSTAB_E_SHAPE, "set_plan_flags: unknown flag bits 0x%x", flags);
+    if ((flags & VSTAB_PLAN_CONV1_ONE_ROW) && (flags & VSTAB_PLAN_CONV1_FORCE_PAIR))
+        return fail(ctx, VSTAB_E_SHAPE, "set_plan_flags: VSTAB_PLAN_CONV1_ONE_ROW and VSTAB_PLAN_CONV1_FORCE_PAIR exclude each other (0x%x)", flags);
     ctx->plan_flags = flags;
     return VSTAB_OK;
 }
diff --git a/coupe/optical_flow_based_deep_video_stabilization_amd/csrc/flownet_plan.h b/coupe/optical_flow_based_deep_video_stabilization_amd/csrc/flownet_plan.h
--- a/coupe/optical_flow_based_deep_video_stabilization_amd/csrc/flownet_plan.h
+++ b/coupe/optical_flow_based_deep_video_stabilization_amd/csrc/flownet_plan.h
@@ -61,6 +61,7 @@
     vstab::ConvTile tile[N_LAYER];
     bool vec4[N_LAYER];
     bool conv1_bf16x3;
+    int conv1_pair;
     bool skinny[N_LAYER];
     bool wino[10];
     vstab::ConvParams wcp[10];
diff --git a/coupe/optical_flow_based_deep_video_stabilization_amd/csrc/rowwin_tile.h b/coupe/optical_flow_based_deep_video_stabilization_amd/csrc/rowwin_tile.h
--- a/coupe/optical_flow_based_deep_video_stabilization_amd/csrc/rowwin_tile.h
+++ b/coupe/optical_flow_based_deep_video_stabilization_amd/csrc/rowwin_tile.h
@@ -22,7 +22,7 @@
 };
 
 template <int MB>
-__device__ __forceinline__ RowWinTile<MB> rowwin_tile(const RowWinParams &p)
+__device__ __forceinline__ RowWinTile<MB> rowwin_tile(const RowWinParams &p, int rows = 1)
 {
     RowWinTile<MB> t;
     t.tid = threadIdx.x;
@@ -33,7 +33,7 @@
     xcd_remap(bx_, by_, bz_);
     if (p.clear_n > 0 && blockIdx.x == 0 && blockIdx.y == 0 && blockIdx.z == 0)
         for (int i = t.tid; i < p.clear_n; i += 256) p.clear_words[i] = 0u;
-    t.row = (int)bx_;
+    t.row = (int)bx_ * rows;
     t.ox0 = p.ox_base + (int)by_ * (64 * MB); t.n = (int)bz_;
     t.pix_step = p.s_in * p.Cs_in;
     t.row_floats = p.Wi * p.Cs_in;
@@ -126,8 +126,8 @@
                                 hipEvent_t ev_stop)
 {
     const int ntx = rowwin_xtiles(q);
-    if (ntx < 0 || ((uintptr_t)q.in & 15) != 0) return hipErrorInvalidValue;
-    dim3 grid(q.stream_rows > 0 ? q.Ho / q.stream_rows : q.Ho, ntx, q.B), block(256);
+    if (ntx < 0 || ((uintptr_t)q.in & 15) != 0 || q.rows < 1 || q.rows > 2) return hipErrorInvalidValue;
+    dim3 grid(q.stream_rows > 0 ? q.Ho / q.stream_rows : (q.Ho + q.rows - 1) / q.rows, ntx, q.B), block(256);
     q.out_vec4 = (((uintptr_t)q.out & 15) == 0 && (q.Cs_out & 3) == 0 && (q.c_off & 3) == 0 && lds >= (size_t)64 * q.MB * 64 * 4) ? 1 : 0;
     const RowWinKernel k = q.MB == 2 ? k72 : k41;
     if (ev_start || ev_stop) hipExtLaunchKernelGGL(k, grid, block, lds, stream, ev_start, ev_stop, 0, q);
diff --git a/coupe/optical_flow_based_deep_video_stabilization_amd/csrc/vstab_internal.h b/coupe/optical_flow_based_deep_video_stabilization_amd/csrc/vstab_internal.h
--- a/coupe/optical_flow_based_deep_video_stabilization_amd/csrc/vstab_internal.h
+++ b/coupe/optical_flow_based_deep_video_stabilization_amd/csrc/vstab_internal.h
@@ -153,6 +153,7 @@
     int Ho, Wo, Cs_out, c_off;
     int N, Npad, act;
     int MB;
+    int rows;
     int out_vec4;
     int asm_loop;
     int stream_rows;
@@ -161,10 +162,11 @@
     int ox_base, ntile_x;
 };
 inline int rowwin_mb(int B, int Ho, int Wo) { return (long long)B * Ho * ((Wo + 127) / 128) < 512 ? 1 : 2; }
+constexpr long long ROWWIN_PAIR_MIN_WORKGROUPS = 2 * 2 * 256;
 inline bool rowwin_geometry_ok(const RowWinParams &p)
 {
     return ((p.s_in * p.Cs_in) % 2 == 0) && ((p.Wi * p.Cs_in) % 4 == 0) && p.N <= 64 && p.Npad == 64 && (p.MB == 1 || p.MB == 2) &&
-           p.WLEN <= (p.MB == 2 ? 7 : 4) * 1024 && (p.WLEN % 4) == 0 && p.in_bytes < 0x80000000u;
+           p.WLEN <= (p.MB == 2 ? 7 : 4) * 1024 && (p.WLEN % 4) == 0 && p.in_bytes < 0x80000000u && (p.rows == 1 || p.rows == 2);
 }
 hipError_t rowwin_set_attributes();
 hipError_t launch_conv_rowwin(const RowWinParams &p, hipStream_t stream, hipEvent_t ev_start = nullptr,
@@ -174,7 +176,10 @@
 void pack_conv_rowwin(const float *W, const double *scale, int kh, int kw, int cin, int cout, int npad,
                       int lead, int segp, float *wpk);
 
-inline bool conv1_bf16x3_geometry_ok(const RowWinParams &p) { return rowwin_geometry_ok(p) && p.KH >= 1 && (p.SEGP % 32) == 0 && p.SEGP >= 32; }
+inline bool conv1_bf16x3_geometry_ok(const RowWinParams &p)
+{
+    return rowwin_geometry_ok(p) && p.KH >= 1 && (p.SEGP % 32) == 0 && p.SEGP >= 32 && (p.rows == 1 || (p.rows == 2 && p.KH > p.s_in && p.s_in >= 1));
+}
 hipError_t conv1_bf16x3_set_attributes();
 hipError_t launch_conv1_bf16x3(const RowWinParams &p, hipStream_t stream, hipEvent_t ev_start = nullptr,
                                hipEvent_t ev_stop = nullptr);
diff --git a/include/vstab.h b/include/vstab.h
--- a/include/vstab.h
+++ b/include/vstab.h
@@ -247,6 +247,8 @@
 #define VSTAB_PLAN_NO_WDEC 8u
 #define VSTAB_PLAN_FORCE_WDEC 16u
 #define VSTAB_PLAN_CONV1_FP32 32u
+#define VSTAB_PLAN_CONV1_ONE_ROW 64u
+#define VSTAB_PLAN_CONV1_FORCE_PAIR 128u
 VSTAB_API int vstab_set_plan_flags(vstab_ctx *ctx, unsigned flags);
 
 VSTAB_API int vstab_conv1_forward(vstab_ctx *ctx, const float *feats, int B, int H, int W, int Cin, float *out, int cs_out, int c_off,
```

New measurement: 2957 frame-pairs/s. 0.987x the previous value.
